# VinAIResearch/Counting-DETR

Measured on AMD Instinct MI355X. Metric: images/sec FSCD-147 2nd-stage train step, higher is better.
Workload: dtype forward bf16x3 (fp32 operands split hi+lo, 3 bf16 MFMAs per product); data / weight gradients bf16 (both operands rounded to bf16, 1 MFMA per product); fp32 accumulate, fp32 storage, fp32 attention softmax / norms / losses / optimizer; 1 GPU; FSCD-147 2nd-stage train step (ResNet-50-DC5 + RCDA enc6/dec6, Q=300 learned, 800x800, T=[37, 120]), fwd+matcher+loss+bwd+clip+AdamW; images_per_gpu=2, global_batch=2, parallelism=dp1, graph=True, precision=bf16x3, precision_backward=bf16, frozen_stage_prefetch=True

## Files before the change

counting_detr_amd/_ffi.py:

```python
import ctypes as C
import os

import torch

_HERE = os.path.dirname(os.path.abspath(__file__))
LIB_PATH = os.environ.get("CDETR_LIB") or os.path.join(_HERE, "lib", "libcdetr_hip.so")

ROWS_DENSE, ROWS_CONV_FWD, ROWS_CONV_DGRAD = 0, 1, 2
_p = C.c_void_p


class ConvGeom(C.Structure):
    _fields_ = [("mode", C.c_int32), ("Ha", C.c_int32), ("Wa", C.c_int32), ("Hc", C.c_int32), ("Wc", C.c_int32),
                ("kh", C.c_int32), ("kw", C.c_int32), ("stride", C.c_int32), ("pad", C.c_int32), ("dil", C.c_int32)]


class GemmDesc(C.Structure):
    _fields_ = [("M", C.c_int32), ("N", C.c_int32), ("K", C.c_int32), ("taps", C.c_int32), ("batch", C.c_int32),
                ("b_layout", C.c_int32), ("relu", C.c_int32), ("precision", C.c_int32), ("out_scale", C.c_float),
                ("A", _p), ("lda", C.c_int64), ("sA", C.c_int64),
                ("B", _p), ("ldb", C.c_int64), ("sB", C.c_int64),
                ("C", _p), ("ldc", C.c_int64), ("sC", C.c_int64),
                ("w_scale", _p), ("bias", _p), ("resid", _p), ("ldr", C.c_int64), ("gate", _p), ("ldg", C.c_int64),
                ("g", ConvGeom), ("B_split", _p), ("batch_inner", C.c_int32), ("flags", C.c_int32),
                ("sA2", C.c_int64), ("sB2", C.c_int64), ("sC2", C.c_int64), ("A16", _p), ("C16", _p),
                ("splitk_ws", _p), ("splitk_ws_bytes", C.c_int64), ("A16lo", _p), ("B16", _p), ("gate16", _p), ("C16lo", _p)]


class WgradDesc(C.Structure):
    _fields_ = [("P", C.c_int32), ("Nout", C.c_int32), ("Cin", C.c_int32), ("taps", C.c_int32), ("batch", C.c_int32), ("precision", C.c_int32),
                ("dY", _p), ("ldy", C.c_int64), ("sY", C.c_int64),
                ("X", _p), ("ldx", C.c_int64), ("sX", C.c_int64),
                ("dW", _p), ("ldw", C.c_int64), ("sW", C.c_int64),
                ("w_scale", _p), ("dbias", _p), ("g", ConvGeom), ("batch_inner", C.c_int32), ("wg_target", C.c_int32),
                ("sY2", C.c_int64), ("sX2", C.c_int64), ("sW2", C.c_int64), ("dY16", _p), ("X16", _p)]


class RcdaFwdDesc(C.Structure):
    _fields_ = [("N", C.c_int32), ("L", C.c_int32), ("H", C.c_int32), ("W", C.c_int32), ("nh", C.c_int32),
                ("precision", C.c_int32), ("scale", C.c_float), ("q_row", _p), ("q_col", _p), ("k_row", _p), ("k_col", _p), ("v", _p),
                ("mask_row", _p), ("mask_col", _p), ("out", _p), ("a_row", _p), ("a_col", _p), ("ws", _p), ("ws_bytes", C.c_int64)]


class RcdaBwdDesc(C.Structure):
    _fields_ = [("N", C.c_int32), ("L", C.c_int32), ("H", C.c_int32), ("W", C.c_int32), ("nh", C.c_int32),
                ("precision", C.c_int32), ("scale", C.c_float), ("d_out", _p), ("a_row", _p), ("a_col", _p), ("v", _p),
                ("ds_row", _p), ("ds_col", _p), ("d_v", _p), ("k_row", _p), ("k_col", _p), ("dq_row", _p), ("dq_col", _p),
                ("q_row", _p), ("q_col", _p), ("dk_row", _p), ("dk_col", _p)]


class AttnDesc(C.Structure):
    _fields_ = [("q", _p), ("k", _p), ("v", _p), ("ldq", C.c_int64), ("ldk", C.c_int64), ("ldv", C.c_int64), ("o", _p), ("lse", _p),
                ("d_o", _p), ("d_q", _p), ("d_k", _p), ("d_v", _p), ("ld_dq", C.c_int64), ("ld_dk", C.c_int64), ("ld_dv", C.c_int64),
                ("work", _p), ("N", C.c_int32), ("Lq", C.c_int32), ("Lk", C.c_int32), ("nh", C.c_int32), ("scale", C.c_float),
                ("precision", C.c_int32)]


class CriterionDesc(C.Structure):
    _fields_ = [("B", C.c_int32), ("Q", C.c_int32), ("C", C.c_int32), ("num_classes", C.c_int32), ("Mmax", C.c_int32), ("alpha", C.c_float),
                ("logits", _p), ("boxes", _p), ("vars", _p), ("tgt_boxes", _p), ("tgt_labels", _p), ("tgt_off", _p), ("idx_i", _p),
                ("idx_j", _p), ("num_boxes", _p), ("losses", _p), ("g_logits", _p), ("g_l1", _p), ("g_giou", _p), ("g_var_box", _p),
                ("g_vars", _p), ("loss_weights", _p)]


class CriterionEvalDesc(C.Structure):
    _fields_ = [("B", C.c_int32), ("Q", C.c_int32), ("C", C.c_int32), ("num_classes", C.c_int32), ("Mmax", C.c_int32), ("alpha", C.c_float),
                ("logits", _p), ("boxes", _p), ("vars", _p), ("tgt_boxes", _p), ("tgt_labels", _p), ("tgt_off", _p), ("idx_i", _p),
                ("idx_j", _p), ("losses", _p), ("loss_weights", _p)]


class MirrorItem(C.Structure):
    _fields_ = [("src", _p), ("dst", _p), ("dst_split", _p), ("scale", _p), ("R", C.c_int32), ("C", C.c_int32), ("taps", C.c_int32),
                ("tile0", C.c_int32), ("transpose", C.c_int32), ("pad_", C.c_int32), ("dst_hi", _p)]


class CocoMatchDesc(C.Structure):
    _fields_ = [("B", C.c_int32), ("A", C.c_int32), ("T", C.c_int32), ("Gtot", C.c_int32), ("Dtot", C.c_int32), ("Gmax", C.c_int32),
                ("gt_boxes", _p), ("gt_area", _p), ("gt_ignore", _p), ("gt_off", _p), ("dt_boxes", _p), ("dt_area", _p), ("dt_off", _p),
                ("iou_thrs", _p), ("area_rng", _p), ("matched", _p), ("det_ignored", _p), ("npig", _p)]


class ImagePrepDesc(C.Structure):
    _fields_ = [("B", C.c_int32), ("Hm", C.c_int32), ("Wm", C.c_int32), ("max_taps", C.c_int32), ("max_rows", C.c_int32), ("pad_", C.c_int32),
                ("pixels", _p), ("pixel_bytes", C.c_int64), ("images", _p), ("tables", _p), ("table_ints", C.c_int64), ("lut", _p),
                ("image", _p), ("mask", _p)]


class EmitDetectionsDesc(C.Structure):
    _fields_ = [("B", C.c_int32), ("Q", C.c_int32), ("N", C.c_int32), ("first", C.c_int32), ("max_det", C.c_int32), ("wire_cap", C.c_int32),
                ("eval_cap", C.c_int32), ("threshold", C.c_float), ("prob", _p), ("boxes", _p), ("points", _p), ("orig_hw", _p), ("counts", _p),
                ("wire_off", _p), ("eval_off", _p), ("wire", _p), ("eval_boxes", _p), ("eval_area", _p), ("eval_score", _p), ("status", _p)]


class EmitPseudoLabelsDesc(C.Structure):
    _fields_ = [("B", C.c_int32), ("R", C.c_int32), ("N", C.c_int32), ("first", C.c_int32), ("max_det", C.c_int32), ("row_cap", C.c_int32),
                ("eval_cap", C.c_int32), ("pad_", C.c_int32), ("points", _p), ("pred_wh", _p), ("counts", _p), ("orig_wh", _p), ("gt_xywh", _p),
                ("img_counts", _p), ("row_off", _p), ("eval_off", _p), ("wire", _p), ("pair_iou", _p), ("eval_boxes", _p), ("eval_area", _p),
                ("eval_score", _p), ("status", _p)]


EXPORTS = ["cdetr_gemm", "cdetr_gemm_dl", "cdetr_gemm_group", "cdetr_wgrad", "cdetr_wgrad_group", "cdetr_colsum", "cdetr_sumsq", "cdetr_adamw_step", "cdetr_adamw_step2", "cdetr_sgd_step", "cdetr_relu_mask", "cdetr_relu_mask2", "cdetr_layernorm_fwd", "cdetr_layernorm_fwd_add", "cdetr_layernorm_bwd", "cdetr_layernorm_bwd_merge", "cdetr_groupnorm_fwd", "cdetr_groupnorm_bwd", "cdetr_groupnorm_fwd_ws", "cdetr_groupnorm_bwd_ws", "cdetr_posadd2",
           "cdetr_hw_reduce", "cdetr_posadd2_hw_reduce", "cdetr_bcast_add2", "cdetr_bcast_add2_sum", "cdetr_add2", "cdetr_grad_merge", "cdetr_sine_embed", "cdetr_sine_embed_bwd", "cdetr_maxpool3x3s2", "cdetr_maxpool3x3s2_split", "cdetr_weight_mirror", "cdetr_weight_images", "cdetr_rcda_fwd", "cdetr_rcda_bwd", "cdetr_mha_fwd", "cdetr_mha_bwd", "cdetr_mha_fwd_lens", "cdetr_mha_bwd_lens", "cdetr_attn_fwd", "cdetr_attn_bwd",
           "cdetr_mask_prep", "cdetr_stem_pack", "cdetr_exemplar_fwd", "cdetr_exemplar_bwd", "cdetr_aggr_weight_fwd", "cdetr_aggr_weight_bwd",
           "cdetr_box_head_fwd", "cdetr_box_head_bwd", "cdetr_match_cost", "cdetr_lsap", "cdetr_criterion_fwd", "cdetr_criterion_bwd", "cdetr_criterion_eval", "cdetr_bbox_criterion_fwd", "cdetr_bbox_criterion_bwd", "cdetr_bbox_criterion_lens_fwd", "cdetr_bbox_criterion_lens_bwd", "cdetr_box_iou_xywh", "cdetr_coco_match", "cdetr_image_prep", "cdetr_emit_detections", "cdetr_emit_pseudo_labels", "cdetr_count_sweep", "cdetr_last_error", "cdetr_abi_version", "cdetr_delay", "cdetr_flag_signal", "cdetr_flag_wait"]

_lib = None


def lib():
    global _lib
    if _lib is None:
        if not os.path.exists(LIB_PATH):
            raise RuntimeError(f"{LIB_PATH} is missing: build it with `python -m counting_detr_amd.build` "
                               "(the Counting-DETR MI355X path has no fallback implementation)")
        L = C.CDLL(LIB_PATH)
        L.cdetr_last_error.restype = C.c_char_p
        L.cdetr_abi_version.restype = C.c_int
        L.cdetr_gemm_dl.restype = C.c_int
        L.cdetr_gemm_dl.argtypes = [_p, C.c_int32, C.c_int32, _p]
        for name in ("cdetr_gemm", "cdetr_wgrad", "cdetr_rcda_fwd", "cdetr_rcda_bwd", "cdetr_attn_fwd", "cdetr_attn_bwd"):
            getattr(L, name).restype = C.c_int
            getattr(L, name).argtypes = [_p, _p]
        L.cdetr_delay.restype = C.c_int
        L.cdetr_delay.argtypes = [C.c_int32, _p]
        L.cdetr_flag_signal.restype = C.c_int
        L.cdetr_flag_signal.argtypes = [_p, _p]
        L.cdetr_flag_wait.restype = C.c_int
        L.cdetr_flag_wait.argtypes = [_p, _p, C.c_int32, C.c_int32, _p]
        L.cdetr_gemm_group.restype = C.c_int
        L.cdetr_gemm_group.argtypes = [_p, C.c_int32, _p]
        L.cdetr_wgrad_group.restype = C.c_int
        L.cdetr_wgrad_group.argtypes = [_p, C.c_int32, _p]
        L.cdetr_colsum.restype = C.c_int
        L.cdetr_colsum.argtypes = [_p, C.c_int64, C.c_int32, C.c_int32, _p, _p]
        L.cdetr_sumsq.restype = C.c_int
        L.cdetr_sumsq.argtypes = [_p, C.c_int64, _p, _p, _p]
        L.cdetr_adamw_step.restype = C.c_int
        L.cdetr_adamw_step.argtypes = [_p, _p, _p, _p, _p, C.c_int64, _p, _p] + [C.c_float] * 6 + [_p]
        L.cdetr_adamw_step2.restype = C.c_int
        L.cdetr_adamw_step2.argtypes = [_p] * 5 + [C.c_float, C.c_float, C.c_int64, C.c_int64, _p, _p] + [C.c_float] * 6 + [_p]
        L.cdetr_sgd_step.restype = C.c_int
        L.cdetr_sgd_step.argtypes = [_p] * 4 + [C.c_float, C.c_float, C.c_int64, C.c_int64, _p, _p] + [C.c_float] * 4 + [_p]
        L.cdetr_relu_mask.restype = C.c_int
        L.cdetr_relu_mask.argtypes = [_p, _p, _p, C.c_int64, C.c_float, _p]
        L.cdetr_relu_mask2.restype = C.c_int
        L.cdetr_relu_mask2.argtypes = [_p, _p, _p, _p, C.c_int64, C.c_float, _p]
        L.cdetr_layernorm_fwd.restype = C.c_int
        L.cdetr_layernorm_fwd.argtypes = [_p] * 6 + [C.c_int32, C.c_int32, C.c_float, _p]
        L.cdetr_layernorm_fwd_add.restype = C.c_int
        L.cdetr_layernorm_fwd_add.argtypes = [_p] * 10 + [C.c_int32, C.c_int32, C.c_float, _p]
        L.cdetr_layernorm_bwd.restype = C.c_int
        L.cdetr_layernorm_bwd.argtypes = [_p] * 9 + [C.c_int32, C.c_int32, _p, _p]
        L.cdetr_layernorm_bwd_merge.restype = C.c_int
        L.cdetr_layernorm_bwd_merge.argtypes = [_p] * 7 + [C.c_float, C.c_float, C.c_int32, C.c_int32] + [_p] * 8 + [C.c_int32, C.c_int32, _p, _p]
        L.cdetr_groupnorm_fwd.restype = C.c_int
        L.cdetr_groupnorm_fwd.argtypes = [_p] * 6 + [C.c_int32] * 4 + [C.c_float, _p]
# ... 108 lines not shown
```

counting_detr_amd/csrc/elementwise.hip:

```cpp
#include "../../include/cdetr_hip.h"
#include "common.h"
#include <stdlib.h>

namespace {

__global__ __launch_bounds__(256) void sumsq_kernel(const float* __restrict__ g, long n, float* __restrict__ ws) {
    float s = 0.f;
    const long n4 = n >> 2;
    const float4* g4 = reinterpret_cast<const float4*>(g);
    for (long i = (long)blockIdx.x * 256 + threadIdx.x; i < n4; i += (long)gridDim.x * 256) {
        const float4 v = g4[i];
        s += v.x * v.x + v.y * v.y + v.z * v.z + v.w * v.w;
    }
    if (blockIdx.x == 0)
        for (long i = (n4 << 2) + threadIdx.x; i < n; i += 256) s += g[i] * g[i];
    s = wave_sum(s);
    __shared__ float part[4];
    if ((threadIdx.x & 63) == 0) part[threadIdx.x >> 6] = s;
    __syncthreads();
    if (threadIdx.x == 0) ws[blockIdx.x] = (part[0] + part[1]) + (part[2] + part[3]);
}

__global__ __launch_bounds__(256) void sumsq_final_kernel(const float* __restrict__ ws, int nblocks, float* __restrict__ out) {
    float t = 0.f;
// ... 72 lines not shown
    if (!clip_coef(sumsq, max_norm, grad_div, coef)) return;
    const long n4 = n >> 2;
    float4* p4 = reinterpret_cast<float4*>(p);
    const float4* g4 = reinterpret_cast<const float4*>(g);
    float4* b4 = reinterpret_cast<float4*>(buf);
    auto upd = [&](float& pp, float gg, float& bb, float l) {
        const float d = gg * coef + wd * pp;
        bb = momentum * bb + d;
        pp -= (l * lr_scale) * bb;
    };
    for (long i = (long)blockIdx.x * 256 + threadIdx.x; i < n4; i += (long)gridDim.x * 256) {
        float4 pp = p4[i], bb = b4[i];
        const float4 gg = g4[i];
        const float4 ll = lr4_at(lr, i, lr0, lr1, lr_split);
        upd(pp.x, gg.x, bb.x, ll.x);
        upd(pp.y, gg.y, bb.y, ll.y);
        upd(pp.z, gg.z, bb.z, ll.z);
        upd(pp.w, gg.w, bb.w, ll.w);
        p4[i] = pp; b4[i] = bb;
    }
    if (blockIdx.x == 0)
        for (long i = (n4 << 2) + threadIdx.x; i < n; i += 256) upd(p[i], g[i], buf[i], lr_at(lr, i, lr0, lr1, lr_split));
}

__global__ void adamw_finish_kernel(const float* __restrict__ sumsq, float* __restrict__ state, float grad_div) {
    const float total_norm = sqrtf(sumsq[0]) * grad_div;
    state[2] = total_norm;
    if (fabsf(total_norm) <= 3.0e38f) state[0] += 1.f;
    else state[3] += 1.f;
}

__global__ __launch_bounds__(256) void relu_mask_kernel(const float* __restrict__ y, const float* __restrict__ dy,
                                                        float* __restrict__ dz, __bf16* __restrict__ dz16, long n, float scale) {
    const long n4 = n >> 2;
    for (long i = (long)blockIdx.x * 256 + threadIdx.x; i < n4; i += (long)gridDim.x * 256) {
        const float4 a = reinterpret_cast<const float4*>(y)[i];
        float4 b = reinterpret_cast<const float4*>(dy)[i];
        b.x = a.x > 0.f ? b.x * scale : 0.f;
        b.y = a.y > 0.f ? b.y * scale : 0.f;
        b.z = a.z > 0.f ? b.z * scale : 0.f;
        b.w = a.w > 0.f ? b.w * scale : 0.f;
        reinterpret_cast<float4*>(dz)[i] = b;
        if (dz16) {
            const f32x2 lo = {b.x, b.y}, hi = {b.z, b.w};
            uint2 t;
            t.x = __builtin_bit_cast(unsigned, __builtin_convertvector(lo, bf16x2));
            t.y = __builtin_bit_cast(unsigned, __builtin_convertvector(hi, bf16x2));
            reinterpret_cast<uint2*>(dz16)[i] = t;
        }
    }
    if (blockIdx.x == 0)
        for (long i = (n4 << 2) + threadIdx.x; i < n; i += 256) {
            const float v = y[i] > 0.f ? dy[i] * scale : 0.f;
            dz[i] = v;
            if (dz16) dz16[i] = (__bf16)v;
        }
}

inline int grid_for(long n4) {
    long b = (n4 + 255) / 256;
    static_assert(CDETR_SUMSQ_MAX_BLOCKS == 2048, "cdetr_sumsq's workspace holds one partial per block of this grid");
    if (b > 2048) b = 2048;
    if (b < 1) b = 1;
    return (int)b;
}


__global__ __launch_bounds__(256) void weight_mirror_kernel(const cdetr_mirror_item* __restrict__ items, const int n_items) {
    __shared__ float tile[32][33];
    const int b = blockIdx.x;
    int lo = 0, hi = n_items - 1;
    while (lo < hi) {
        const int mid = (lo + hi + 1) >> 1;
        if (items[mid].tile0 <= b) lo = mid; else hi = mid - 1;
    }
    const cdetr_mirror_item it = items[lo];
    const int tilesC = (it.C + 31) >> 5, tilesR = (it.R + 31) >> 5;
    int t = b - it.tile0;
    const int tap = t / (tilesR * tilesC);
    t -= tap * tilesR * tilesC;
    const int r0 = (t / tilesC) * 32, c0 = (t % tilesC) * 32;
    const int tx = threadIdx.x & 31, ty = threadIdx.x >> 5;
    __bf16* sp = reinterpret_cast<__bf16*>(it.dst_split);
    float vin[4], sin_[4];
    const int cc = min(c0 + tx, it.C - 1);
#pragma unroll
    for (int p = 0; p < 4; ++p) vin[p] = it.src[((long)min(r0 + ty + 8 * p, it.R - 1) * it.taps + tap) * it.C + cc];
    if (it.scale) {
#pragma unroll
        for (int p = 0; p < 4; ++p) sin_[p] = it.scale[min(r0 + ty + 8 * p, it.R - 1)];
    } else {
#pragma unroll
        for (int p = 0; p < 4; ++p) sin_[p] = 1.f;
    }
#pragma unroll
    for (int p = 0; p < 4; ++p) {
        const int r = r0 + ty + 8 * p, c = c0 + tx;
        const float v = (r < it.R && c < it.C) ? (it.scale ? vin[p] * sin_[p] : vin[p]) : 0.f;
        tile[ty + 8 * p][tx] = v;
        if (!it.transpose && sp && r < it.R && c < it.C) {
            const __bf16 h = (__bf16)v;
            __bf16* g = sp + (long)r * it.taps * it.C * 2 + (long)((tap * it.C + c0) >> 5) * 64;
            g[tx] = h;
            g[32 + tx] = (__bf16)(v - (float)h);
        }
    }
    if (!it.transpose) return;
    __syncthreads();
#pragma unroll
    for (int p = 0; p < 4; ++p) {
        const int c = c0 + ty + 8 * p, r = r0 + tx;
        if (r < it.R && c < it.C) {
            const float v = tile[tx][ty + 8 * p];
            if (it.dst) it.dst[((long)c * it.taps + tap) * it.R + r] = v;
            if (it.dst_hi) reinterpret_cast<__bf16*>(it.dst_hi)[((long)c * it.taps + tap) * it.R + r] = (__bf16)v;
            if (sp) {
                const __bf16 h = (__bf16)v;
                __bf16* g = sp + (long)c * it.taps * it.R * 2 + (long)((tap * it.R + r0) >> 5) * 64;
                g[tx] = h;
                g[32 + tx] = (__bf16)(v - (float)h);
            }
        }
    }
}
constexpr int WIMG_BLOCK = 4096;
__global__ __launch_bounds__(256) void weight_image_kernel(const cdetr_mirror_item* __restrict__ items, const int n_items) {
    const int b = blockIdx.x;
    int lo = 0, hi = n_items - 1;
    while (lo < hi) {
        const int mid = (lo + hi + 1) >> 1;
        if (items[mid].tile0 <= b) lo = mid; else hi = mid - 1;
    }
    const cdetr_mirror_item it = items[lo];
    const long K = (long)it.taps * it.C, total = (long)it.R * K;
    const long e0 = (long)(b - it.tile0) * WIMG_BLOCK + threadIdx.x * 4;
    __bf16* sp = reinterpret_cast<__bf16*>(it.dst_split);
    const bool al = (reinterpret_cast<uintptr_t>(it.src) & 15) == 0;
    float4 v[4];
    float sc[4];
#pragma unroll
    for (int u = 0; u < 4; ++u) {
        const long e = min(e0 + u * 1024, total - 4);
        if (al) v[u] = *reinterpret_cast<const float4*>(it.src + e);
        else v[u] = make_float4(it.src[e], it.src[e + 1], it.src[e + 2], it.src[e + 3]);
        sc[u] = it.scale ? it.scale[e / K] : 1.f;
    }
#pragma unroll
    for (int u = 0; u < 4; ++u) {
        const long e = e0 + u * 1024;
        if (e >= total) continue;
        const float x[4] = {it.scale ? v[u].x * sc[u] : v[u].x, it.scale ? v[u].y * sc[u] : v[u].y, it.scale ? v[u].z * sc[u] : v[u].z,
                            it.scale ? v[u].w * sc[u] : v[u].w};
        __bf16 h[4], l[4];
#pragma unroll
        for (int j = 0; j < 4; ++j) {
            h[j] = (__bf16)x[j];
            l[j] = (__bf16)(x[j] - (float)h[j]);
        }
        __bf16* g = sp + (e >> 5) * 64 + (e & 31);
        *reinterpret_cast<uint2*>(g) = *reinterpret_cast<const uint2*>(h);
        *reinterpret_cast<uint2*>(g + 32) = *reinterpret_cast<const uint2*>(l);
    }
}

template <int NT>
__device__ __forceinline__ float block_sum(float v, float* red) {
    v = wave_sum(v);
    const int lane = threadIdx.x & 63, wid = threadIdx.x >> 6;
    __syncthreads();
    if (lane == 0) red[wid] = v;
    __syncthreads();
    float t = 0.f;
#pragma unroll
    for (int i = 0; i < NT / 64; ++i) t += red[i];
    return t;
}
constexpr int GN_NT = 1024;
constexpr int GN_NT_BWD = 256;

__global__ __launch_bounds__(GN_NT) void gn_fwd_kernel(const float* __restrict__ x, const float* __restrict__ gamma,
                                                     const float* __restrict__ beta, float* __restrict__ y, float* __restrict__ mean,
                                                     float* __restrict__ rstd, int P, int C, int G, float eps) {
    __shared__ float red[GN_NT / 64];
    const int CG = C / G, q4 = CG >> 2;
    const int b = blockIdx.x / G, g = blockIdx.x % G;
    const float* xb = x + (long)b * P * C + g * CG;
    float* yb = y + (long)b * P * C + g * CG;
    const int n4 = P * q4;
    float s1 = 0.f, s2 = 0.f;
    for (int i = threadIdx.x; i < n4; i += GN_NT) {
        const int p = i / q4, c4 = i - p * q4;
        const float4 v = *reinterpret_cast<const float4*>(xb + (long)p * C + c4 * 4);
        s1 += (v.x + v.y) + (v.z + v.w);
    }
    const float inv = 1.f / ((float)P * CG);
    const float mu = block_sum<GN_NT>(s1, red) * inv;
    for (int i = threadIdx.x; i < n4; i += GN_NT) {
        const int p = i / q4, c4 = i - p * q4;
        const float4 v = *reinterpret_cast<const float4*>(xb + (long)p * C + c4 * 4);
        const float a = v.x - mu, b2 = v.y - mu, c2 = v.z - mu, e2 = v.w - mu;
        s2 += (a * a + b2 * b2) + (c2 * c2 + e2 * e2);
// ... 928 lines not shown
```

counting_detr_amd/csrc/igemm.hip:

```cpp
#include "../../include/cdetr_hip.h"
#include "common.h"
#include "rows.h"
#include <stdlib.h>
#include <type_traits>
#include <vector>
#include <algorithm>

namespace {

constexpr int BK = 16;
constexpr int LDS_K = BK + 4;

__device__ __forceinline__ float4 ld4(const float* p) { return *reinterpret_cast<const float4*>(p); }
typedef unsigned u32x4 __attribute__((ext_vector_type(4)));
__device__ __forceinline__ u32x4 ld16(const __bf16* p) { return *reinterpret_cast<const u32x4*>(p); }
__device__ __forceinline__ float4 zero4() { return make_float4(0.f, 0.f, 0.f, 0.f); }

template <int BM, int BN, int BL>
__global__ __launch_bounds__(256) void igemm_kernel(const cdetr_gemm_desc d, const int tilesM, const int vecA,
                                                    const int vecB) {
    constexpr int FM = BM / 64, FN = BN / 64;
    constexpr int A_SLOTS = BM / 64, B_SLOTS = BN / 64;
    constexpr int LDS_N = BN + 4;
    constexpr int B_TILE = (BL == 0) ? BN * LDS_K : BK * LDS_N;
// ... 1518 lines not shown
            const int k = k0 + u * 16 + g4 * 4;
            if constexpr (VA) {
                const float4 t = ld4(arow + (k < kend ? k : 0));
                a[u][0] = t.x; a[u][1] = t.y; a[u][2] = t.z; a[u][3] = t.w;
            } else {
#pragma unroll
                for (int s = 0; s < 4; ++s) a[u][s] = arow[k + s < kend ? k + s : 0];
            }
            if (BL == 0) {
                if constexpr (VB) {
                    const float4 t = ld4(brow + (k < kend ? k : 0));
                    b[u][0] = t.x; b[u][1] = t.y; b[u][2] = t.z; b[u][3] = t.w;
                } else {
#pragma unroll
                    for (int s = 0; s < 4; ++s) b[u][s] = brow[k + s < kend ? k + s : 0];
                }
            } else {
#pragma unroll
                for (int s = 0; s < 4; ++s) {
                    const int kk = k + s < kend ? k + s : 0;
                    b[u][s] = brow[(long)kk * d.ldb];
                    bw[u][s] = wsp[wsc ? kk : 0];
                }
            }
        }
        __builtin_amdgcn_sched_barrier(0);
#pragma unroll
        for (int u = 0; u < UB; ++u) {
            const int k = k0 + u * 16 + g4 * 4;
#pragma unroll
            for (int s = 0; s < 4; ++s) {
                const bool oka = VA ? (k < kend) : (k + s < kend);
                const bool okb = (BL == 0 && VB) ? (k < kend) : (k + s < kend);
                a[u][s] *= oka ? am : 0.f;
                if (BL == 0) b[u][s] *= okb ? bm : 0.f;
                else b[u][s] = (okb && nv) ? (wsc ? b[u][s] * bw[BL == 0 ? 0 : u][s] : b[u][s]) : 0.f;
            }
        }
#pragma unroll
        for (int u = 0; u < UB; ++u)
#pragma unroll
            for (int s = 0; s < 4; ++s) acc = __builtin_amdgcn_mfma_f32_16x16x4f32(a[u][s], b[u][s], acc, 0, 0, 0);
    }
    };
    using T_ = std::true_type;
    using F_ = std::false_type;
    if (vecA) { if (vecB || BL != 0) run(T_{}, T_{}); else run(T_{}, F_{}); }
    else { if (vecB || BL != 0) run(F_{}, T_{}); else run(F_{}, F_{}); }
    mfma_drain(acc);
#pragma unroll
    for (int r = 0; r < 4; ++r) red[wid][r * 64 + lane] = acc[r];
    __syncthreads();
    if (wid != 0) return;
    const int no = tn * 16 + i;
    if (no >= d.N) return;
#pragma unroll
    for (int r = 0; r < 4; ++r) {
        const int mo = tm * 16 + g4 * 4 + r;
        if (mo >= d.M) continue;
        const float sum = (red[0][r * 64 + lane] + red[1][r * 64 + lane]) + (red[2][r * 64 + lane] + red[3][r * 64 + lane]);
        float v = (sum + bias) * d.out_scale + rv[r];
        v = gv[r] > 0.f ? v : 0.f;
        if (d.relu) v = fmaxf(v, 0.f);
        C[(long)mo * d.ldc + no] = v;
        if (C16) C16[(long)mo * d.ldc + no] = (__bf16)v;
    }
}

template <int BL, int UB>
__global__ __launch_bounds__(256) void igemm_direct_kernel(const cdetr_gemm_desc d, const int tilesM, const int tilesN,
                                                           const int vecA, const int vecB) {
    igemm_direct_body<BL, UB>(d, tilesM, tilesN, vecA, vecB, blockIdx.x, blockIdx.z);
}

template <int BL, int UB>
__global__ __launch_bounds__(256) void igemm_direct_group_kernel(const GemmGroupArgs g) {
    int p = 0;
    while (p + 1 < g.n && (int)blockIdx.x >= g.blk0[p + 1]) ++p;
    const GemmGroupItem& it = g.it[p];
    const int lb = blockIdx.x - g.blk0[p];
    igemm_direct_body<BL, UB>(it.d, it.tilesM, it.tilesN, it.vecA, it.vecB, lb % it.nx, lb / it.nx);
}

template <int TERMS>
__global__ __launch_bounds__(512) void igemm_mixed_group_kernel(const GemmGroupArgs g) {
    int p = 0;
    while (p + 1 < g.n && (int)blockIdx.x >= g.blk0[p + 1]) ++p;
    const GemmGroupItem& it = g.it[p];
    const int lb = blockIdx.x - g.blk0[p];
    if (it.pad_ == 0) {
        if (threadIdx.x >= 256) return;
        igemm_direct_body<0, 4>(it.d, it.tilesM, it.tilesN, it.vecA, it.vecB, lb % it.nx, lb / it.nx);
    } else {
        igemm_fast_body<2, 4, 1, 1, 0, 32, 3, TERMS>(it.d, it.tilesM, lb % it.nx, lb / it.nx);
    }
}

__device__ __forceinline__ void wgrad_direct_body(const cdetr_wgrad_desc& d, const int tilesI, const int tilesJ, const int p_per_slice,
                                                  float* __restrict__ dbias, const int bx, const int by, const int bz, const bool single) {
    constexpr int UB = 8;
    const int wid = threadIdx.x >> 6, lane = threadIdx.x & 63;
    const int tile = bx * 4 + wid;
    if (tile >= tilesI * tilesJ) return;
    const int ti = tile % tilesI, tj = tile / tilesI;
    const int i = lane & 15, g4 = lane >> 4;
    const int z = bz;
    const float* __restrict__ dY = d.dY + batch_off(z, d.batch_inner, d.sY, d.sY2);
    const float* __restrict__ X = d.X + batch_off(z, d.batch_inner, d.sX, d.sX2);
    float* __restrict__ dW = d.dW + batch_off(z, d.batch_inner, d.sW, d.sW2);
    const int ci = ti * 16 + i, cc = tj * 16 + i;
    const bool iv = ci < d.Nout, cv = cc < d.Cin;
    const float* ya = dY + (iv ? ci : 0);
    const float* xb = X + (cv ? cc : 0);
    const float fa = iv ? 1.f : 0.f, fb = cv ? 1.f : 0.f;
    const int pbeg = by * p_per_slice, pend = min(d.P, pbeg + p_per_slice);
    float ws[4] = {1.f, 1.f, 1.f, 1.f};
    if (d.w_scale) {
#pragma unroll
        for (int r = 0; r < 4; ++r) ws[r] = d.w_scale[min(ti * 16 + g4 * 4 + r, d.Nout - 1)];
    }
    f32x4 acc = {0.f, 0.f, 0.f, 0.f};
    float bsum = 0.f;
    for (int p0 = pbeg; p0 < pend; p0 += 16 * UB) {
        float a[UB][4], b[UB][4];
#pragma unroll
        for (int u = 0; u < UB; ++u)
#pragma unroll
            for (int s = 0; s < 4; ++s) {
                const int p = p0 + u * 16 + g4 * 4 + s;
                const bool pv = p < pend;
                const long pc = pv ? p : 0;
                a[u][s] = ya[pc * d.ldy] * (pv ? fa : 0.f);
                b[u][s] = xb[pc * d.ldx] * (pv ? fb : 0.f);
            }
#pragma unroll
        for (int u = 0; u < UB; ++u)
#pragma unroll
            for (int s = 0; s < 4; ++s) {
                acc = __builtin_amdgcn_mfma_f32_16x16x4f32(a[u][s], b[u][s], acc, 0, 0, 0);
                bsum += a[u][s];
            }
    }
    mfma_drain(acc);
    const int co = tj * 16 + i;
    if (co < d.Cin) {
#pragma unroll
        for (int r = 0; r < 4; ++r) {
            const int io = ti * 16 + g4 * 4 + r;
            if (io >= d.Nout) continue;
            const float v = acc[r] * ws[r];
            float* dst = dW + (long)io * d.ldw + co;
            if (single) *dst += v;
            else atomicAdd(dst, v);
        }
    }
    if (dbias != nullptr && tj == 0) {
        bsum += __shfl_xor(bsum, 16, 64);
        bsum = xhalf_sum(bsum);
        if (g4 == 0 && iv) atomicAdd(dbias + ci, bsum);
    }
}

__global__ __launch_bounds__(256) void wgrad_direct_kernel(const cdetr_wgrad_desc d, const int tilesI, const int tilesJ,
                                                           const int p_per_slice, float* __restrict__ dbias) {
    wgrad_direct_body(d, tilesI, tilesJ, p_per_slice, dbias, blockIdx.x, blockIdx.y, blockIdx.z, gridDim.y == 1);
}
// ... 284 lines not shown
        const int tilesM = (d.M + 15) / 16, tilesN = (d.N + 15) / 16;
        dim3 grid(tilesM * tilesN, 1, d.batch);
        const int cpw = (((d.K + 15) >> 4) + 3) >> 2;
        auto go = [&](auto k0, auto k1) {
            if (d.b_layout == 0) hipLaunchKernelGGL(k0, grid, dim3(256), 0, st, d, tilesM, tilesN, vecA, vecB);
            else hipLaunchKernelGGL(k1, grid, dim3(256), 0, st, d, tilesM, tilesN, vecA, vecB);
        };
        if (cpw <= 4) go(igemm_direct_kernel<0, 4>, igemm_direct_kernel<1, 4>);
        else if (cpw <= 8) go(igemm_direct_kernel<0, 8>, igemm_direct_kernel<1, 8>);
        else go(igemm_direct_kernel<0, 16>, igemm_direct_kernel<1, 16>);
        return cdetr_launch_status("cdetr_gemm");
    }
    if (vecA && vecB && (d.K % 32) == 0) {
        if (gemm_is_f44(d)) {
            if (d.splitk_ws && d.batch == 1 && blocks(128, 128) < 224 && (long)d.K * d.taps >= 4096) return launch_gemm_fast<2, 4, 2, 1, 32>(d, st);
            if (blocks(128, 128) < 224 && blocks(96, 128) <= 256) return launch_gemm_fast<3, 4, 1, 1, 32>(d, st);
            return launch_gemm_fast<4, 4, 1, 1, 32>(d, st);
        }
        if (gemm_is_f24(d)) return launch_gemm_fast<2, 4, 1, 1, 32>(d, st);
        if ((d.K % 64) == 0 && blocks(64, 64) < 512) return launch_gemm_fast<2, 2, 1, 1, 64>(d, st);
        return launch_gemm_fast<2, 2, 1, 1, 32>(d, st);
    }
    if (d.N > 64 && d.M > 64 && blocks(128, 128) >= 384) return launch_gemm<128, 128>(d, st, vecA, vecB);
    if (d.M > 64 && blocks(128, 64) >= 384) return launch_gemm<128, 64>(d, st, vecA, vecB);
    return launch_gemm<64, 64>(d, st, vecA, vecB);
}

extern "C" int cdetr_gemm_group(const cdetr_gemm_desc* descs, int32_t n, void* stream) {
    CDETR_CHECK_ARG(n >= 0 && (descs != nullptr || n == 0), "cdetr_gemm_group: bad arguments");
    hipStream_t st = reinterpret_cast<hipStream_t>(stream);
    const char* force_s = cdetr_tune_env("CDETR_GEMM_VARIANT");
    const bool grouping = !(force_s && atoi(force_s) != 0);
    std::vector<int> cls[5];
    for (int i = 0; i < n; ++i) {
        const cdetr_gemm_desc& d = descs[i];
        if (int rcv = check_gemm_desc(d)) return rcv;
        if (d.M == 0) continue;
        const int vecA = gemm_vec_a(d), vecB = gemm_vec_b(d);
        int c = -1;
        if (grouping && gemm_is_direct(d, vecA, vecB)) {
            if (d.b_layout == 0) {
                const int cpw = (((d.K + 15) >> 4) + 3) >> 2;
                c = cpw <= 4 ? 0 : (cpw <= 8 ? 1 : 2);
            }
        } else if (grouping && vecA && vecB && (d.K % 32) == 0 && !gemm_is_f44(d) && gemm_is_f24(d) && d.B_split && d.batch == 1) {
            c = d.precision == 3 ? 4 : 3;
        }
        if (c >= 0) cls[c].push_back(i);
        else if (int rc1 = cdetr_gemm(&d, stream)) return rc1;
    }
    const int tc = !cls[3].empty() ? 3 : 4;
    if (!cls[0].empty() && (cls[3].empty() != cls[4].empty()) && cls[0].size() + cls[tc].size() <= (size_t)GG_MAX) {
        GemmGroupArgs g;
        int m = 0;
        g.blk0[0] = 0;
        for (int pass = 0; pass < 2; ++pass) {
            for (int idx : (pass == 0 ? cls[tc] : cls[0])) {
                GemmGroupItem& it = g.it[m];
                it.d = descs[idx];
                it.vecA = gemm_vec_a(it.d); it.vecB = gemm_vec_b(it.d); it.pad_ = pass == 0 ? 1 : 0;
                if (pass == 1) {
                    it.tilesM = (it.d.M + 15) / 16; it.tilesN = (it.d.N + 15) / 16;
                    it.nx = it.tilesM * it.tilesN;
                } else {
                    it.tilesM = (it.d.M + 63) / 64; it.tilesN = (it.d.N + 127) / 128;
                    it.nx = 8 * ((it.tilesM + 7) / 8) * it.tilesN;
                }
                g.blk0[m + 1] = g.blk0[m] + it.nx * it.d.batch;
                ++m;
            }
        }
        g.n = m;
        const int bytes = (2 * 64 * 36 + 2 * 128 * 36) * 4;
        if (tc == 3) {
            if (int rcl = raise_lds(igemm_mixed_group_kernel<3>, bytes, "cdetr_gemm_group")) return rcl;
            hipLaunchKernelGGL(igemm_mixed_group_kernel<3>, dim3(g.blk0[m]), dim3(512), bytes, st, g);
        } else {
            if (int rcl = raise_lds(igemm_mixed_group_kernel<1>, bytes, "cdetr_gemm_group")) return rcl;
            hipLaunchKernelGGL(igemm_mixed_group_kernel<1>, dim3(g.blk0[m]), dim3(512), bytes, st, g);
        }
        if (int rcl = cdetr_launch_status("cdetr_gemm_group")) return rcl;
        cls[0].clear();
        cls[tc].clear();
    }
    for (int c = 0; c < 5; ++c) {
        for (size_t c0 = 0; c0 < cls[c].size(); c0 += GG_MAX) {
            const int m = (int)std::min<size_t>(GG_MAX, cls[c].size() - c0);
            if (m == 1) { if (int rc1 = cdetr_gemm(&descs[cls[c][c0]], stream)) return rc1; continue; }
            GemmGroupArgs g;
            g.n = m; g.blk0[0] = 0;
            for (int k = 0; k < m; ++k) {
                GemmGroupItem& it = g.it[k];
                it.d = descs[cls[c][c0 + k]];
                it.vecA = gemm_vec_a(it.d); it.vecB = gemm_vec_b(it.d); it.pad_ = 0;
                if (c < 3) {
                    it.tilesM = (it.d.M + 15) / 16; it.tilesN = (it.d.N + 15) / 16;
                    it.nx = it.tilesM * it.tilesN;
                } else {
                    it.tilesM = (it.d.M + 63) / 64; it.tilesN = (it.d.N + 127) / 128;
                    it.nx = 8 * ((it.tilesM + 7) / 8) * it.tilesN;
                }
                g.blk0[k + 1] = g.blk0[k] + it.nx * it.d.batch;
            }
            if (c == 0) hipLaunchKernelGGL((igemm_direct_group_kernel<0, 4>), dim3(g.blk0[m]), dim3(256), 0, st, g);
            else if (c == 1) hipLaunchKernelGGL((igemm_direct_group_kernel<0, 8>), dim3(g.blk0[m]), dim3(256), 0, st, g);
            else if (c == 2) hipLaunchKernelGGL((igemm_direct_group_kernel<0, 16>), dim3(g.blk0[m]), dim3(256), 0, st, g);
            else if (c == 3) {
                const int bytes = (2 * 64 * 36 + 2 * 128 * 36) * 4;
                if (int rcl = raise_lds(igemm_fast_group_kernel<2, 4, 1, 1, 0, 32, 3>, bytes, "cdetr_gemm_group")) return rcl;
                hipLaunchKernelGGL((igemm_fast_group_kernel<2, 4, 1, 1, 0, 32, 3>), dim3(g.blk0[m]), dim3(512), bytes, st, g);
            } else {
                const int bytes = (2 * 64 * 36 + 2 * 128 * 36) * 4;
                if (int rcl = raise_lds(igemm_fast_group_kernel<2, 4, 1, 1, 0, 32, 3, 1>, bytes, "cdetr_gemm_group")) return rcl;
                hipLaunchKernelGGL((igemm_fast_group_kernel<2, 4, 1, 1, 0, 32, 3, 1>), dim3(g.blk0[m]), dim3(512), bytes, st, g);
            }
            if (int rcl = cdetr_launch_status("cdetr_gemm_group")) return rcl;
        }
    }
    return CDETR_OK;
}

namespace {
bool wgrad_has_twins(const cdetr_wgrad_desc& d);
bool wgrad_is_direct(const cdetr_wgrad_desc& d);
bool wgrad_is_fast(const cdetr_wgrad_desc& d);
int check_wgrad_desc(const cdetr_wgrad_desc& d) {
    CDETR_CHECK_ARG(d.P >= 0 && d.Nout > 0 && d.Cin > 0 && d.taps > 0 && d.batch > 0, "cdetr_wgrad: bad sizes");
    CDETR_CHECK_ARG((d.dY || d.dY16) && (d.X || d.X16) && d.dW, "cdetr_wgrad: null pointer");
    CDETR_CHECK_ARG((d.dY && d.X) || (wgrad_has_twins(d) && wgrad_is_fast(d) && !wgrad_is_direct(d)),
                    "cdetr_wgrad: dY == NULL / X == NULL need dY16 + X16, plain-bf16 products and a problem of the tile-kernel class");
    CDETR_CHECK_ARG(aligned16(d.dY) && aligned16(d.X) && (d.sY & 3) == 0 && (d.sX & 3) == 0 && (d.sY2 & 3) == 0 && (d.sX2 & 3) == 0, "cdetr_wgrad: dY/X must be 16-byte aligned");
    if (d.g.mode == CDETR_ROWS_DENSE) {
        CDETR_CHECK_ARG(d.taps == 1, "cdetr_wgrad: dense rows need taps == 1");
    } else {
        CDETR_CHECK_ARG(d.g.mode == CDETR_ROWS_CONV_FWD && d.taps == d.g.kh * d.g.kw, "cdetr_wgrad: geometry");
        CDETR_CHECK_ARG(d.P % (d.g.Hc * d.g.Wc) == 0, "cdetr_wgrad: P is not images*Hc*Wc");
    }
    return CDETR_OK;
}
void direct_wgrad_plan(const cdetr_wgrad_desc& d, int& tilesI, int& tilesJ, int& per, int& slices) {
    tilesI = (d.Nout + 15) / 16; tilesJ = (d.Cin + 15) / 16;
    slices = (d.P + 127) / 128;
    if (slices > 8) slices = 8;
    per = (d.P + slices - 1) / slices;
    per = ((per + 15) / 16) * 16;
    slices = (d.P + per - 1) / per;
}
bool wgrad_is_direct(const cdetr_wgrad_desc& d) {
    return d.g.mode == CDETR_ROWS_DENSE && (d.P <= 256 || !((d.ldy & 3) == 0 && (d.ldx & 3) == 0 && (d.Nout & 3) == 0 && (d.Cin & 3) == 0)) && d.P <= 1024;
}
bool wgrad_has_twins(const cdetr_wgrad_desc& d) {
    return d.precision == 3 && d.dY16 && d.X16 && !d.dbias && (d.Nout & 7) == 0 && (d.Cin & 7) == 0 && (d.ldy & 7) == 0 && (d.ldx & 7) == 0 &&
           (d.sY & 7) == 0 && (d.sX & 7) == 0 && (d.sY2 & 7) == 0 && (d.sX2 & 7) == 0 && aligned16(d.dY16) && aligned16(d.X16) && d.Nout >= 8 && d.Cin >= 8;
}
int wgrad_kp() {
    const char* e = cdetr_tune_env("CDETR_WGRAD_KP");
    const int kp = e ? atoi(e) : 1;
    return kp >= 4 ? 4 : kp >= 2 ? 2 : 1;
}
bool wgrad_is_fast(const cdetr_wgrad_desc& d) { return (d.ldy & 3) == 0 && (d.ldx & 3) == 0 && (d.Nout & 3) == 0 && (d.Cin & 3) == 0; }
}

extern "C" int cdetr_wgrad(const cdetr_wgrad_desc* dp, void* stream) {
    CDETR_CHECK_ARG(dp != nullptr, "cdetr_wgrad: null descriptor");
    cdetr_wgrad_desc d = *dp;
    if (int rcv = check_wgrad_desc(d)) return rcv;
// ... 224 lines not shown
```

counting_detr_amd/csrc/rcda.hip:

```cpp
#include "../../include/cdetr_hip.h"
#include "common.h"
#include <algorithm>
#include <type_traits>
#include <stdlib.h>

namespace {

__device__ __forceinline__ void xcd_slab(int& bx, int& by) {
    const int gx = gridDim.x, total = gx * gridDim.y;
    if (total & 7) return;
    const int lin = by * gx + bx;
    const int l2 = (lin & 7) * (total >> 3) + (lin >> 3);
    by = l2 / gx;
    bx = l2 - by * gx;
}


constexpr int D = 32;
constexpr int QW = 32;

__device__ __forceinline__ float4 ld4(const float* p) { return *reinterpret_cast<const float4*>(p); }

struct FwdSmem {
    int sw, sh;
// ... 879 lines not shown
        if (!PROBE && nq > 0 && d.ds_col) save_rows(Acol, sm.sh, d.ds_col + (((long)n * d.nh + head) * L + qbase) * Hp, nq, Hp, lane);
    }
    stamp(3);
    float qv[2][2][8];
    if (PREC == 1 && d.dq_row && d.dk_row) {
#pragma unroll
        for (int side = 0; side < 2; ++side)
#pragma unroll
            for (int st = 0; st < 2; ++st)
#pragma unroll
                for (int j = 0; j < 8; ++j) {
                    const int qq = qbase + 16 * st + 8 * g + j;
                    qv[side][st][j] = (side == 0 ? d.q_row : d.q_col)[((long)n * L + min(max(qq, 0), L - 1)) * E + head * D + i32];
                }
    }
    if (d.dq_row) {
        float* Kk = smem + sm.off_kk;
        if (kpre_ok) {
#pragma unroll
            for (int u = 0; u < KP; ++u) {
                const int idx = tid + NT * u;
                if (idx < nk8) *reinterpret_cast<float4*>(Kk + (idx >> 3) * D + (idx & 7) * 4) = kpre[u];
            }
        } else
        for (int base = 0; base < nk8; base += 4 * NT) {
            float4 t[4];
#pragma unroll
            for (int u = 0; u < 4; ++u) {
                const int idx = min(base + tid + NT * u, nk8 - 1);
                const int key = idx >> 3, c4 = idx & 7;
                const float* src = (key < W) ? d.k_row + ((long)n * W + key) * E + head * D + c4 * 4
                                             : d.k_col + ((long)n * H + (key - W)) * E + head * D + c4 * 4;
                t[u] = ld4(src);
            }
#pragma unroll
            for (int u = 0; u < 4; ++u) {
                const int idx = base + tid + NT * u;
                if (idx < nk8) *reinterpret_cast<float4*>(Kk + (idx >> 3) * D + (idx & 7) * 4) = t[u];
            }
        }
        __syncthreads();
        stamp(4);
        if constexpr (PREC == 1) {
#pragma unroll
            for (int side = 0; side < 2; ++side) {
                const int nkeys = side == 0 ? W : H;
                const float* S = side == 0 ? dArow + i32 * sm.sw : Acol + i32 * sm.sh;
                const float* Ks = Kk + (side == 0 ? 0 : W * D) + i32;
                f32x16 acc = {0.f, 0.f, 0.f, 0.f, 0.f, 0.f, 0.f, 0.f, 0.f, 0.f, 0.f, 0.f, 0.f, 0.f, 0.f, 0.f};
                const int nks = (nkeys + 15) >> 4;
                for (int st = 0; st < nks; ++st) {
                    float a[8], b[8];
#pragma unroll
                    for (int j = 0; j < 8; ++j) {
                        const int w = 16 * st + 8 * g + j;
                        const int wc = min(w, nkeys - 1);
                        const float av = Ks[wc * D], bv = S[wc];
                        a[j] = (w < nkeys) ? av : 0.f;
                        b[j] = (w < nkeys) ? bv : 0.f;
                    }
                    bf16x8 ah, al, bh, bl;
                    split_bf16x8(a, ah, al);
                    split_bf16x8(b, bh, bl);
                    acc = mfma_bf16_terms<TERMS>(ah, al, bh, bl, acc);
                }
                mfma_drain(acc);
                if (qvalid) {
                    float* dst = (side == 0 ? d.dq_row : d.dq_col) + ((long)n * L + q) * E + head * D + 4 * g;
#pragma unroll
                    for (int j = 0; j < 4; ++j)
                        *reinterpret_cast<float4*>(dst + 8 * j) = make_float4(acc[4 * j], acc[4 * j + 1], acc[4 * j + 2], acc[4 * j + 3]);
                }
            }
            stamp(5);
            if (d.dk_row) {
                const bool wg_reduce = W <= 128 && H <= 128;
                constexpr int NTL = 4;
#pragma unroll
                for (int side = 0; side < 2; ++side) {
                    const int nkeys = side == 0 ? W : H;
                    const float* S = side == 0 ? dArow : Acol;
                    float* Sw = side == 0 ? dArow : Acol;
                    const int sstr = side == 0 ? sm.sw : sm.sh;
                    float* acc_g = (side == 0 ? d.dk_row + (long)n * W * E : d.dk_col + (long)n * H * E) + head * D + i32;
                    bf16x8 bh[2], bl[2];
#pragma unroll
                    for (int st = 0; st < 2; ++st) {
                        float b[8];
#pragma unroll
                        for (int j = 0; j < 8; ++j) b[j] = (qbase + 16 * st + 8 * g + j < L) ? qv[side][st][j] : 0.f;
                        split_bf16x8(b, bh[st], bl[st]);
                    }
                    const int ntile = (nkeys + 31) >> 5;
                    auto tile = [&](int tl) __attribute__((always_inline)) -> f32x16 {
                        const int wkey = 32 * tl + i32, wc = min(wkey, nkeys - 1);
                        f32x16 acc = {0.f, 0.f, 0.f, 0.f, 0.f, 0.f, 0.f, 0.f, 0.f, 0.f, 0.f, 0.f, 0.f, 0.f, 0.f, 0.f};
#pragma unroll
                        for (int st = 0; st < 2; ++st) {
                            float a[8];
#pragma unroll
                            for (int j = 0; j < 8; ++j) {
                                const float av = S[(16 * st + 8 * g + j) * sstr + wc];
                                a[j] = (wkey < nkeys) ? av : 0.f;
                            }
                            bf16x8 ah, al;
                            split_bf16x8(a, ah, al);
                            acc = mfma_bf16_terms<TERMS>(ah, al, bh[st], bl[st], acc);
                        }
                        mfma_drain(acc);
                        return acc;
                    };
                    if (wg_reduce) {
                        f32x16 accs[NTL];
#pragma unroll
                        for (int tl = 0; tl < NTL; ++tl)
                            if (tl < ntile) accs[tl] = tile(tl);
                        wave_sync();
#pragma unroll
                        for (int tl = 0; tl < NTL; ++tl)
                            if (tl < ntile) {
#pragma unroll
                                for (int r = 0; r < 16; ++r) {
                                    const int wk = 32 * tl + (r & 3) + 8 * (r >> 2) + 4 * g;
                                    Sw[min(wk, nkeys) * D + i32] = accs[tl][r];
                                }
                            }
                    } else {
                        for (int tl = 0; tl < ntile; ++tl) {
                            const f32x16 acc = tile(tl);
#pragma unroll
                            for (int r = 0; r < 16; ++r) {
                                const int wk = 32 * tl + (r & 3) + 8 * (r >> 2) + 4 * g;
                                if (wk < nkeys) atomicAdd(acc_g + (long)wk * E, acc[r]);
                            }
                        }
                    }
                }
                if (wg_reduce) {
                    __syncthreads();
                    const int nrow = W * D, ntot = (W + H) * D;
                    for (int e = tid; e < ntot; e += NT) {
                        const bool rowside = e < nrow;
                        const int idx = rowside ? e : e - nrow;
                        const float* base = rowside ? smem + sm.off_r + idx : smem + sm.off_u + idx;
                        const int wstr = rowside ? QW * sm.sw : QW * sm.su;
                        float sum = 0.f;
#pragma unroll
                        for (int wv = 0; wv < NW; ++wv) sum += base[wv * wstr];
                        const int key = idx >> 5, ch = idx & 31;
                        float* dst = rowside ? d.dk_row + ((long)n * W + key) * E + head * D + ch : d.dk_col + ((long)n * H + key) * E + head * D + ch;
                        atomicAdd(dst, sum);
                    }
                }
            }
            stamp(6);
            flush_probe();
            return;
        }
#pragma unroll
        for (int side = 0; side < 2; ++side) {
            const int nkeys = side == 0 ? W : H;
            const float* S = side == 0 ? dArow + i32 * sm.sw : Acol + i32 * sm.sh;
            const float* Ks = Kk + (side == 0 ? 0 : W * D) + 16 * g;
            float acc[16];
#pragma unroll
            for (int j = 0; j < 16; ++j) acc[j] = 0.f;
#pragma unroll 2
            for (int k = 0; k < nkeys; ++k) {
                const float a = S[k];
#pragma unroll
                for (int c4 = 0; c4 < 4; ++c4) {
                    const float4 kv = *reinterpret_cast<const float4*>(Ks + k * D + c4 * 4);
                    acc[c4 * 4 + 0] = fmaf(a, kv.x, acc[c4 * 4 + 0]);
                    acc[c4 * 4 + 1] = fmaf(a, kv.y, acc[c4 * 4 + 1]);
                    acc[c4 * 4 + 2] = fmaf(a, kv.z, acc[c4 * 4 + 2]);
                    acc[c4 * 4 + 3] = fmaf(a, kv.w, acc[c4 * 4 + 3]);
                }
            }
            if (qvalid) {
                float* dst = (side == 0 ? d.dq_row : d.dq_col) + ((long)n * L + q) * E + head * D + 16 * g;
#pragma unroll
                for (int c4 = 0; c4 < 4; ++c4)
                    *reinterpret_cast<float4*>(dst + c4 * 4) = make_float4(acc[c4 * 4], acc[c4 * 4 + 1], acc[c4 * 4 + 2], acc[c4 * 4 + 3]);
            }
        }
    }
}

template <int NF, int NW, int PREC, int TERMS = 3, bool PROBE = false>
__global__ __launch_bounds__(64 * NW) void rcda_bwd_kernel(const cdetr_rcda_bwd_desc d) {
    int bx_ = blockIdx.x, by_ = blockIdx.y;
    xcd_slab(bx_, by_);
    rcda_bwd_body<NF, NW, PREC, TERMS, PROBE>(d, bx_, by_);
}

template <int NF, int PREC>
__global__ __launch_bounds__(256) void rcda_dv_kernel(const cdetr_rcda_bwd_desc d, const int q_per_slice) {
    constexpr int QT = 64;
    constexpr int HR = 32 * NF;
    extern __shared__ __attribute__((aligned(16))) float smem[];
    const int H = d.H, W = d.W, L = d.L, E = d.nh * D;
    const int Wp = (W + 3) & ~3, Hp = (H + 7) & ~7;
    float* Ac = smem;
    float* Ar = Ac + QT * HR;
    float* Do = Ar + QT * Wp;
    const int tid = threadIdx.x, lane = tid & 63, wid = tid >> 6;
    const int i32 = lane & 31, g = lane >> 5;
    const int n = blockIdx.y / d.nh, head = blockIdx.y % d.nh;
    const int w = blockIdx.x * 4 + wid;
    const bool wvalid = w < W;
    const int qs = blockIdx.z * q_per_slice;
    const int qe = min(L, qs + q_per_slice);
    const float* gac = d.a_col + ((long)n * d.nh + head) * L * Hp;
    const float* gar = d.a_row + ((long)n * d.nh + head) * L * Wp;
    const float* gdo = d.d_out + (long)n * L * E + head * D;

    f32x16 acc[NF];
#pragma unroll
    for (int f = 0; f < NF; ++f)
#pragma unroll
        for (int r = 0; r < 16; ++r) acc[f][r] = 0.f;

    for (int q0 = qs; q0 < qe; q0 += QT) {
        const int nq = min(QT, qe - q0);
        __syncthreads();
        for (int idx = tid; idx < QT * HR; idx += 256) {
            const int r = idx / HR, c = idx - r * HR;
            Ac[idx] = (r < nq && c < Hp) ? gac[(long)(q0 + r) * Hp + c] : 0.f;
        }
        for (int idx = tid; idx < QT * Wp; idx += 256) {
            const int r = idx / Wp;
            Ar[idx] = (r < nq) ? gar[(long)q0 * Wp + idx] : 0.f;
        }
        for (int idx = tid; idx < QT * 8; idx += 256) {
            const int r = idx >> 3, c4 = idx & 7;
            *reinterpret_cast<float4*>(Do + r * D + c4 * 4) =
                (r < nq) ? ld4(gdo + (long)(q0 + r) * E + c4 * 4) : make_float4(0.f, 0.f, 0.f, 0.f);
        }
        __syncthreads();
        if (wvalid && PREC == 0) {
#pragma unroll 2
            for (int kk = 0; kk < QT / 8; ++kk) {
#pragma unroll
                for (int s = 0; s < 4; ++s) {
                    const int qq = kk * 8 + g * 4 + s;
                    const float ar = Ar[qq * Wp + w];
                    const float b = Do[qq * D + i32];
#pragma unroll
                    for (int f = 0; f < NF; ++f) {
                        const float a = Ac[qq * HR + 32 * f + i32] * ar;
                        acc[f] = __builtin_amdgcn_mfma_f32_32x32x2f32(a, b, acc[f], 0, 0, 0);
                    }
                }
            }
        }
        if (wvalid && PREC == 1) {
#pragma unroll 2
            for (int kp = 0; kp < QT / 16; ++kp) {
                float arv[8], bv[8];
                int qs[8];
#pragma unroll
                for (int t = 0; t < 4; ++t) {
                    qs[t] = (2 * kp) * 8 + g * 4 + t;
                    qs[4 + t] = (2 * kp + 1) * 8 + g * 4 + t;
                }
#pragma unroll
                for (int t = 0; t < 8; ++t) {
                    arv[t] = Ar[qs[t] * Wp + w];
                    bv[t] = Do[qs[t] * D + i32];
                }
                bf16x8 bh, bl;
                split_bf16x8(bv, bh, bl);
#pragma unroll
                for (int f = 0; f < NF; ++f) {
                    float av[8];
#pragma unroll
                    for (int t = 0; t < 8; ++t) av[t] = Ac[qs[t] * HR + 32 * f + i32] * arv[t];
                    bf16x8 ah, al;
                    split_bf16x8(av, ah, al);
                    acc[f] = mfma_bf16x3(ah, al, bh, bl, acc[f]);
                }
            }
        }
    }
    mfma_drain(acc);
    if (!wvalid) return;
#pragma unroll
    for (int f = 0; f < NF; ++f)
#pragma unroll
        for (int r = 0; r < 16; ++r) {
            const int h = 32 * f + (r & 3) + 8 * (r >> 2) + 4 * g;
            if (h < H) atomicAdd(d.d_v + (((long)n * H + h) * W + w) * E + head * D + i32, acc[f][r]);
        }
}

struct Dv2Smem { int art, dot, act, tile, total; };
__host__ __device__ inline Dv2Smem dv2_smem() {
    Dv2Smem s;
    s.art = 0;
    s.dot = 64 * 68;
    s.act = s.dot + 32 * 68;
    s.tile = s.act + 8 * 68;
    s.total = 2 * s.tile;
    return s;
}

template <int TERMS = 3>
__device__ __forceinline__ void rcda_dv2_body(const cdetr_rcda_bwd_desc& d, const int q_per_slice, const int bx, const int by, const int bz) {
    constexpr int QT = 64, ARS = 136;
    extern __shared__ __attribute__((aligned(16))) float smem[];
    const Dv2Smem sm = dv2_smem();
    const int H = d.H, W = d.W, L = d.L, E = d.nh * D;
    const int Wp = (W + 3) & ~3, Hp = (H + 7) & ~7;
    const int tid = threadIdx.x, lane = tid & 63, wid = tid >> 6;
    const int i32 = lane & 31, g = lane >> 5;
    const int n = by / d.nh, head = by % d.nh;
    const int nhg = (H + 7) >> 3;
    const int wchunk = bx / nhg;
    const int nwc = (Wp + 63) >> 6;
    const int wper = (((Wp + nwc - 1) / nwc) + 3) & ~3;
    const int wbase = wchunk * wper;
    const int Wc = min(wper, Wp - wbase);
    const int h0 = (bx - wchunk * nhg) * 8, h = h0 + wid;
    const int qs = bz * q_per_slice;
    const int qe = min(L, qs + q_per_slice);
    const int ntile = (qe - qs + QT - 1) / QT;
    if (ntile <= 0) return;

    const int nrb = 16 * (Wc >> 2);
    int role, q4, x4;
    if (tid < nrb) { role = 0; q4 = tid & 15; x4 = tid >> 4; }
    else if (tid >= 256 && tid < 384) { role = 1; q4 = (tid - 256) & 15; x4 = (tid - 256) >> 4; }
    else if (tid >= 384 && tid < 416) { role = 2; q4 = (tid - 384) & 15; x4 = (tid - 384) >> 4; }
    else { role = 3; q4 = 0; x4 = 0; }
    const float* src;
    long rstride;
    if (role == 0) { src = d.a_row + (((long)n * d.nh + head) * L) * Wp + wbase + x4 * 4; rstride = Wp; }
    else if (role == 1) { src = d.d_out + (long)n * L * E + head * D + x4 * 4; rstride = E; }
    else { src = d.a_col + (((long)n * d.nh + head) * L) * Hp + min(h0 + x4 * 4, Hp - 4); rstride = Hp; }
    float4 rs[2][4];
    unsigned rmask[2] = {0, 0};
    int tf = 0;
    auto fetch = [&](float4 (&r)[4], unsigned& m) __attribute__((always_inline)) {
        const int qb = qs + min(tf, ntile - 1) * QT + q4 * 4;
        m = 0;
#pragma unroll
        for (int kk = 0; kk < 4; ++kk) {
            const int q = qb + kk;
            r[kk] = ld4(src + (long)min(q, L - 1) * rstride);
            m |= (q < qe ? 1u : 0u) << kk;
        }
        ++tf;
    };
    auto stash = [&](const float4 (&r0)[4], unsigned m, int buf) __attribute__((always_inline)) {
        float4 r[4];
#pragma unroll
        for (int kk = 0; kk < 4; ++kk) r[kk] = ((m >> kk) & 1u) ? r0[kk] : make_float4(0.f, 0.f, 0.f, 0.f);
        float* base = smem + buf * sm.tile;
        if (role == 0) {
            __bf16* dst = reinterpret_cast<__bf16*>(base + sm.art) + (x4 * 4) * ARS + q4 * 4;
            stash_split4(dst, 64, r[0].x, r[1].x, r[2].x, r[3].x);
            stash_split4(dst + ARS, 64, r[0].y, r[1].y, r[2].y, r[3].y);
            stash_split4(dst + 2 * ARS, 64, r[0].z, r[1].z, r[2].z, r[3].z);
            stash_split4(dst + 3 * ARS, 64, r[0].w, r[1].w, r[2].w, r[3].w);
        } else if (role == 1 || role == 2) {
            float* dst = base + (role == 1 ? sm.dot : sm.act) + (x4 * 4) * 68 + q4 * 4;
            *reinterpret_cast<float4*>(dst) = make_float4(r[0].x, r[1].x, r[2].x, r[3].x);
            *reinterpret_cast<float4*>(dst + 68) = make_float4(r[0].y, r[1].y, r[2].y, r[3].y);
            *reinterpret_cast<float4*>(dst + 2 * 68) = make_float4(r[0].z, r[1].z, r[2].z, r[3].z);
            *reinterpret_cast<float4*>(dst + 3 * 68) = make_float4(r[0].w, r[1].w, r[2].w, r[3].w);
        }
    };
    for (int idx = tid; idx < 2 * (64 - Wc) * (ARS / 2); idx += 512) {
        const int b = idx / ((64 - Wc) * (ARS / 2)), r = idx - b * (64 - Wc) * (ARS / 2);
        smem[b * sm.tile + sm.art + Wc * (ARS / 2) + r] = 0.f;
    }

    f32x16 acc[2];
#pragma unroll
    for (int f = 0; f < 2; ++f)
#pragma unroll
        for (int r = 0; r < 16; ++r) acc[f][r] = 0.f;

    auto compute = [&](int buf) __attribute__((always_inline)) {
        const float* base = smem + buf * sm.tile;
        const __bf16* art = reinterpret_cast<const __bf16*>(base + sm.art) + i32 * ARS + 8 * g;
        const float* dot = base + sm.dot + i32 * 68 + 8 * g;
        const float* act = base + sm.act + wid * 68 + 8 * g;
#pragma unroll
        for (int ks = 0; ks < 4; ++ks) {
            const float4 d0 = *reinterpret_cast<const float4*>(dot + 16 * ks), d1 = *reinterpret_cast<const float4*>(dot + 16 * ks + 4);
            const float4 a0 = *reinterpret_cast<const float4*>(act + 16 * ks), a1 = *reinterpret_cast<const float4*>(act + 16 * ks + 4);
            const float x[8] = {d0.x * a0.x, d0.y * a0.y, d0.z * a0.z, d0.w * a0.w, d1.x * a1.x, d1.y * a1.y, d1.z * a1.z, d1.w * a1.w};
            bf16x8 bh, bl;
            split_bf16x8(x, bh, bl);
#pragma unroll
            for (int f = 0; f < 2; ++f) {
                const bf16x8 ah = *reinterpret_cast<const bf16x8*>(art + 32 * f * ARS + 16 * ks);
                const bf16x8 al = *reinterpret_cast<const bf16x8*>(art + 32 * f * ARS + 64 + 16 * ks);
                acc[f] = mfma_bf16_terms<TERMS>(ah, al, bh, bl, acc[f]);
            }
        }
    };

    fetch(rs[0], rmask[0]);
    fetch(rs[1], rmask[1]);
    __syncthreads();
    stash(rs[0], rmask[0], 0);
    __syncthreads();
    int t = 0;
    for (; t + 1 < ntile; t += 2) {
        fetch(rs[0], rmask[0]);
        compute(0);
        stash(rs[1], rmask[1], 1);
        __syncthreads();
        fetch(rs[1], rmask[1]);
        compute(1);
        stash(rs[0], rmask[0], 0);
        __syncthreads();
    }
    if (t < ntile) compute(0);
    mfma_drain(acc);
    if (h >= H) return;
#pragma unroll
    for (int f = 0; f < 2; ++f)
#pragma unroll
        for (int r = 0; r < 16; ++r) {
            const int wl = 32 * f + (r & 3) + 8 * (r >> 2) + 4 * g, w = wbase + wl;
            if (wl < Wc && w < W) atomicAdd(d.d_v + (((long)n * H + h) * W + w) * E + head * D + i32, acc[f][r]);
        }
}

template <int TERMS = 3>
__global__ __launch_bounds__(512) void rcda_dv2_kernel(const cdetr_rcda_bwd_desc d, const int q_per_slice) {
    int bx_ = blockIdx.x, by_ = blockIdx.y;
    xcd_slab(bx_, by_);
    rcda_dv2_body<TERMS>(d, q_per_slice, bx_, by_, blockIdx.z);
}

template <int NF, int NW, int TERMS>
__global__ __launch_bounds__(512) void rcda_bwd_all_kernel(const cdetr_rcda_bwd_desc d, const int nqb, const int hgroups, const int q_per_slice) {
    int bx_ = blockIdx.x, by_ = blockIdx.y;
    xcd_slab(bx_, by_);
    if (bx_ < nqb) {
        if ((int)threadIdx.x >= 64 * NW) return;
        rcda_bwd_body<NF, NW, 1, TERMS>(d, bx_, by_);
    } else {
        const int t = bx_ - nqb;
        rcda_dv2_body<TERMS>(d, q_per_slice, t % hgroups, by_, t / hgroups);
    }
}

template <typename F>
int set_smem(F func, int bytes, const char* what) {
    if (bytes > 160 * 1024) {
        cdetr_set_error("%s: needs %d bytes of LDS (> 160 KiB): feature map too large for this tiling", what, bytes);
        return CDETR_ERR_UNSUPPORTED;
    }
    if (bytes > 64 * 1024) {
        hipError_t e = hipFuncSetAttribute(reinterpret_cast<const void*>(func), hipFuncAttributeMaxDynamicSharedMemorySize, bytes);
        if (e != hipSuccess) {
            cdetr_set_error("%s: hipFuncSetAttribute(%d): %s", what, bytes, hipGetErrorString(e));
            return CDETR_ERR_LAUNCH;
        }
    }
    return CDETR_OK;
}

template <int NF>
int launch_rcda_fwd(const cdetr_rcda_fwd_desc& d, hipStream_t st) {
    constexpr int NW = 4;
    const FwdSmem sm = fwd_smem(d.H, d.W, NW);
    const int bytes = sm.total * 4;
    int rc;
    dim3 grid((d.L + QW * NW - 1) / (QW * NW), d.N * d.nh), block(64 * NW);
    if (d.precision == 1) {
        if ((rc = set_smem(rcda_fwd_kernel<NF, NW, 1>, bytes, "cdetr_rcda_fwd"))) return rc;
        hipLaunchKernelGGL((rcda_fwd_kernel<NF, NW, 1>), grid, block, bytes, st, d);
    } else {
        if ((rc = set_smem(rcda_fwd_kernel<NF, NW, 0>, bytes, "cdetr_rcda_fwd"))) return rc;
        hipLaunchKernelGGL((rcda_fwd_kernel<NF, NW, 0>), grid, block, bytes, st, d);
    }
    return cdetr_launch_status("cdetr_rcda_fwd");
}
template <int NF, int NW>
int launch_rcda_bwd_all(const cdetr_rcda_bwd_desc& d, hipStream_t st, int hgroups, int slices, int per) {
    const int bytes = std::max(bwd_smem(d.H, d.W, NF, NW, d.dq_row != nullptr).total * 4, dv2_smem().total * 4);
    int rc;
    const int nqb = (d.L + QW * NW - 1) / (QW * NW);
    dim3 grid(nqb + hgroups * slices, d.N * d.nh);
    if (d.precision == 3) {
        if ((rc = set_smem(rcda_bwd_all_kernel<NF, NW, 1>, bytes, "cdetr_rcda_bwd"))) return rc;
        hipLaunchKernelGGL((rcda_bwd_all_kernel<NF, NW, 1>), grid, dim3(512), bytes, st, d, nqb, hgroups, per);
    } else {
        if ((rc = set_smem(rcda_bwd_all_kernel<NF, NW, 3>, bytes, "cdetr_rcda_bwd"))) return rc;
        hipLaunchKernelGGL((rcda_bwd_all_kernel<NF, NW, 3>), grid, dim3(512), bytes, st, d, nqb, hgroups, per);
    }
    return cdetr_launch_status("cdetr_rcda_bwd(dS+dV)");
}
template <int NF, int NW>
int launch_rcda_bwd(const cdetr_rcda_bwd_desc& d, hipStream_t st) {
    const BwdSmem sm = bwd_smem(d.H, d.W, NF, NW, d.dq_row != nullptr);
    const int bytes = sm.total * 4;
    int rc;
    dim3 grid((d.L + QW * NW - 1) / (QW * NW), d.N * d.nh), block(64 * NW);
    if constexpr (NF == 4) {
        if (d.precision == 3) {
            if ((rc = set_smem(rcda_bwd_kernel<NF, NW, 1, 1>, bytes, "cdetr_rcda_bwd"))) return rc;
            hipLaunchKernelGGL((rcda_bwd_kernel<NF, NW, 1, 1>), grid, block, bytes, st, d);
            return cdetr_launch_status("cdetr_rcda_bwd(dS)");
        }
        if (d.precision >= 1) {
            if ((rc = set_smem(rcda_bwd_kernel<NF, NW, 1>, bytes, "cdetr_rcda_bwd"))) return rc;
            hipLaunchKernelGGL((rcda_bwd_kernel<NF, NW, 1>), grid, block, bytes, st, d);
            return cdetr_launch_status("cdetr_rcda_bwd(dS)");
        }
    }
    if ((rc = set_smem(rcda_bwd_kernel<NF, NW, 0>, bytes, "cdetr_rcda_bwd"))) return rc;
    hipLaunchKernelGGL((rcda_bwd_kernel<NF, NW, 0>), grid, block, bytes, st, d);
    return cdetr_launch_status("cdetr_rcda_bwd(dS)");
}
inline bool rcda_wg5(int L, int NH) {
    const long wg4 = (long)((L + QW * 4 - 1) / (QW * 4)) * NH, wg5 = (long)((L + QW * 5 - 1) / (QW * 5)) * NH;
    return wg4 > 256 && wg4 <= 512 && wg5 <= 256;
}
inline int fwd2_slices(const cdetr_rcda_fwd_desc& d, int base, int nt, int lds_bytes) {
    if (!d.ws || base > RCDA_WS_COUNTERS) return 1;
    int hs;
    const char* f = cdetr_tune_env("CDETR_RCDA_HS");
    if (f) hs = atoi(f);
    else {
        const int per_cu = lds_bytes > 0 ? std::max(1, std::min(4, (160 * 1024) / lds_bytes)) : 1;
        (void)per_cu;
        hs = 256 / base;
    }
    hs = std::min(std::min(hs, 8), d.H / 8);
    const long avail = (long)d.ws_bytes - (long)RCDA_WS_COUNTERS * 4;
    while (hs > 1 && (long)base * hs * 16 * nt * 4 > avail) --hs;
    return hs < 1 ? 1 : hs;
}
inline int rcda_probe() {
    const char* p = cdetr_tune_env("CDETR_RCDA_PROBE");
    return p ? atoi(p) : 0;
}

}

extern "C" int cdetr_rcda_fwd(const cdetr_rcda_fwd_desc* dp, void* stream) {
    CDETR_CHECK_ARG(dp != nullptr, "cdetr_rcda_fwd: null descriptor");
    const cdetr_rcda_fwd_desc d = *dp;
    CDETR_CHECK_ARG(d.N > 0 && d.L > 0 && d.H > 0 && d.W > 0 && d.nh > 0, "cdetr_rcda_fwd: bad sizes");
    CDETR_CHECK_ARG(d.H <= 128 && d.W <= 1024, "cdetr_rcda_fwd: H must be <= 128 (got %d)", d.H);
    CDETR_CHECK_ARG(d.q_row && d.q_col && d.k_row && d.k_col && d.v && d.out, "cdetr_rcda_fwd: null pointer");
    CDETR_CHECK_ARG((d.a_row != nullptr) == (d.a_col != nullptr), "cdetr_rcda_fwd: a_row and a_col are saved together or not at all (both NULL: inference)");
    hipStream_t st = reinterpret_cast<hipStream_t>(stream);
    if (d.precision == 1 && d.W <= 96) {
        const int ks = (d.W + 15) / 16;
        auto go = [&](auto kern, int NWv, int KSv = 0, bool sliced = true) -> int {
            const FwdSmem sm = fwd_smem(d.H, d.W, NWv);
            const int bytes = fwd2_smem(sm, d.H, d.W, KSv ? KSv : ks).total * 4;
            int rc;
            if ((rc = set_smem(kern, bytes, "cdetr_rcda_fwd"))) return rc;
            dim3 grid((d.L + QW * NWv - 1) / (QW * NWv), d.N * d.nh), block(64 * NWv);
            if (sliced) grid.z = fwd2_slices(d, (int)(grid.x * grid.y), 64 * NWv, bytes);
            hipLaunchKernelGGL(kern, grid, block, bytes, st, d);
            return cdetr_launch_status("cdetr_rcda_fwd");
        };
        if (const int probe = rcda_probe(); probe && d.ws && ks == 4 && d.H <= 64)
            return probe == 5 ? go(rcda_fwd2_kernel<5, 4, 2, true>, 5, 0, false) : go(rcda_fwd2_kernel<4, 4, 2, true>, 4, 0, false);
        if (ks == 4 && rcda_wg5(d.L, d.N * d.nh)) return go(rcda_fwd2_kernel<5, 4>, 5);
        if (ks > 4 || d.H > 64) {
            if (d.H > 64 && d.H <= 96) return ks <= 4 ? go(rcda_fwd2_kernel<4, 4, 3>, 4, 4) : go(rcda_fwd2_kernel<4, 6, 3>, 4, 6);
            if (ks <= 4) return go(rcda_fwd2_kernel<4, 4>, 4, 4);
            return ks == 5 ? go(rcda_fwd2_kernel<4, 5>, 4) : go(rcda_fwd2_kernel<4, 6>, 4);
        }
        if (ks == 1) return go(rcda_fwd2_kernel<4, 1>, 4);
        if (ks == 2) return go(rcda_fwd2_kernel<4, 2>, 4);
        if (ks == 3) return go(rcda_fwd2_kernel<4, 3>, 4);
        return go(rcda_fwd2_kernel<4, 4>, 4);
    }
    if (d.H <= 32) return launch_rcda_fwd<1>(d, st);
    if (d.H <= 64) return launch_rcda_fwd<2>(d, st);
    return launch_rcda_fwd<4>(d, st);
}

extern "C" int cdetr_rcda_bwd(const cdetr_rcda_bwd_desc* dp, void* stream) {
    CDETR_CHECK_ARG(dp != nullptr, "cdetr_rcda_bwd: null descriptor");
    const cdetr_rcda_bwd_desc d = *dp;
    CDETR_CHECK_ARG(d.N > 0 && d.L > 0 && d.H > 0 && d.W > 0 && d.nh > 0, "cdetr_rcda_bwd: bad sizes");
    CDETR_CHECK_ARG(d.H <= 128 && d.W <= 1024, "cdetr_rcda_bwd: H must be <= 128 (got %d)", d.H);
    CDETR_CHECK_ARG(d.d_out && d.a_row && d.a_col && d.v && d.d_v, "cdetr_rcda_bwd: null pointer");
    CDETR_CHECK_ARG((d.ds_row && d.ds_col) || (!d.ds_row && !d.ds_col && d.dk_row),
                    "cdetr_rcda_bwd: ds_row / ds_col may only be omitted (both) when the fused q / k gradients are requested");
    CDETR_CHECK_ARG(!d.dq_row || (d.dq_col && d.k_row && d.k_col), "cdetr_rcda_bwd: dq_row needs dq_col, k_row and k_col");
    CDETR_CHECK_ARG(!d.dk_row || (d.dq_row && d.dk_col && d.q_row && d.q_col && d.precision >= 1),
                    "cdetr_rcda_bwd: dk_row needs dk_col, q_row, q_col, the dq_* outputs and a split-bf16 precision (1 or 3)");
    hipStream_t st = reinterpret_cast<hipStream_t>(stream);
    const int NF = d.H <= 32 ? 1 : (d.H <= 64 ? 2 : 4);
    const int Wp = (d.W + 3) & ~3;
    int rc;
    if (const int probe = rcda_probe(); probe && NF == 2 && d.precision == 3 && d.ds_row && d.dk_row) {
        const int NWp = probe == 5 ? 5 : 4;
        const BwdSmem sm = bwd_smem(d.H, d.W, 2, NWp, true);
        dim3 grid((d.L + QW * NWp - 1) / (QW * NWp), d.N * d.nh), block(64 * NWp);
        if (NWp == 5) {
            if ((rc = set_smem(rcda_bwd_kernel<2, 5, 1, 1, true>, sm.total * 4, "cdetr_rcda_bwd"))) return rc;
            hipLaunchKernelGGL((rcda_bwd_kernel<2, 5, 1, 1, true>), grid, block, sm.total * 4, st, d);
        } else {
            if ((rc = set_smem(rcda_bwd_kernel<2, 4, 1, 1, true>, sm.total * 4, "cdetr_rcda_bwd"))) return rc;
            hipLaunchKernelGGL((rcda_bwd_kernel<2, 4, 1, 1, true>), grid, block, sm.total * 4, st, d);
        }
        return cdetr_launch_status("cdetr_rcda_bwd(probe)");
    }
    const bool wg5 = NF == 2 && rcda_wg5(d.L, d.N * d.nh);
    const bool dv2 = d.precision >= 1;
    if (dv2) {
        const int hgroups = ((d.H + 7) / 8) * ((Wp + 63) / 64);
        const long base = (long)hgroups * d.N * d.nh;
        const long ds_wgs = (long)((d.L + QW * 4 - 1) / (QW * 4)) * d.N * d.nh;
        const int dv2_target = ds_wgs <= 128 ? 112 : 224;
        int slices = (int)((dv2_target + base - 1) / base);
        const int max_slices = (d.L + 255) / 256;
        if (slices > max_slices) slices = max_slices;
        if (slices < 1) slices = 1;
        int per = (d.L + slices - 1) / slices;
        per = ((per + 63) / 64) * 64;
        slices = (d.L + per - 1) / per;
        if (NF == 1) return launch_rcda_bwd_all<1, 4>(d, st, hgroups, slices, per);
        if (NF == 2) return wg5 ? launch_rcda_bwd_all<2, 5>(d, st, hgroups, slices, per) : launch_rcda_bwd_all<2, 4>(d, st, hgroups, slices, per);
        if ((rc = launch_rcda_bwd<4, 4>(d, st))) return rc;
        const int bytes = dv2_smem().total * 4;
        if (d.precision == 3) {
            if ((rc = set_smem(rcda_dv2_kernel<1>, bytes, "cdetr_rcda_bwd(dV)"))) return rc;
            hipLaunchKernelGGL(rcda_dv2_kernel<1>, dim3(hgroups, d.N * d.nh, slices), dim3(512), bytes, st, d, per);
        } else {
            if ((rc = set_smem(rcda_dv2_kernel<3>, bytes, "cdetr_rcda_bwd(dV)"))) return rc;
            hipLaunchKernelGGL(rcda_dv2_kernel<3>, dim3(hgroups, d.N * d.nh, slices), dim3(512), bytes, st, d, per);
        }
        return cdetr_launch_status("cdetr_rcda_bwd(dV)");
    }
    if (NF == 1) rc = launch_rcda_bwd<1, 4>(d, st);
    else if (NF == 2) rc = wg5 ? launch_rcda_bwd<2, 5>(d, st) : launch_rcda_bwd<2, 4>(d, st);
    else rc = launch_rcda_bwd<4, 4>(d, st);
    if (rc) return rc;
    const int bytes = (64 * 32 * NF + 64 * Wp + 64 * 32) * 4;
    const int wgroups = (d.W + 3) / 4;
    const long base = (long)wgroups * d.N * d.nh;
    int slices = (int)((1024 + base - 1) / base);
    const int max_slices = (d.L + 127) / 128;
    if (slices > max_slices) slices = max_slices;
    if (slices < 1) slices = 1;
    int per = (d.L + slices - 1) / slices;
    per = ((per + 63) / 64) * 64;
    slices = (d.L + per - 1) / per;
    dim3 grid(wgroups, d.N * d.nh, slices), block(256);
    auto dv = [&](auto kern) -> int {
        if ((rc = set_smem(kern, bytes, "cdetr_rcda_bwd(dV)"))) return rc;
        hipLaunchKernelGGL(kern, grid, block, bytes, st, d, per);
        return cdetr_launch_status("cdetr_rcda_bwd(dV)");
    };
    if (NF == 1) return dv(rcda_dv_kernel<1, 0>);
    if (NF == 2) return dv(rcda_dv_kernel<2, 0>);
    return dv(rcda_dv_kernel<4, 0>);
}
```

counting_detr_amd/engine.py:

```python
import math
import os
import sys

import torch
import torch.distributed as dist

from . import backbone as _bb
from .misc import NestedTensor, get_world_size, is_dist_avail_and_initialized, nested_tensor_from_tensor_list, reduce_dict

UNUSED_PREFIXES = ("input_proj.",)


def _segment_of(name):
    if "backbone" in name:
        for li in (4, 3, 2):
            if f"layer{li}." in name:
                return {4: 1, 3: 2, 2: 3}[li]
        return 3
    return 0


class FlatGradExchange:

    def __init__(self, flat_g, seg_bounds):
# ... 77 lines not shown
                if g is not None:
                    g.replay()
                else:
                    self.works.append(dist.all_reduce(buf, async_op=True))
        elif self.stream is not None:
            ev = torch.cuda.Event()
            ev.record(torch.cuda.current_stream())
            self.stream.wait_event(ev)
            if also is not None:
                self.stream.wait_stream(also)
            with torch.cuda.stream(self.stream):
                b0 = mark(self.stream)
                if g is not None:
                    g.replay()
                else:
                    dist.all_reduce(buf)
                b1 = mark(self.stream)
            if self.trace is not None:
                self.trace["buckets"].append((seg, b0, b1))
        else:
            dist.all_reduce(buf)

    def finish(self):
        nseg = len(self.seg_bounds) - 1
        for seg in range(nseg):
            if seg not in self.launched:
                self.segment_done(seg)
        self.launched = []
        if self.stream is not None:
            cur = torch.cuda.current_stream()
            if self.on_side:
                ea = eb = None
                if self.probe is not None:
                    ea, eb = torch.cuda.Event(enable_timing=True), torch.cuda.Event(enable_timing=True)
                    ea.record(cur)
                for w in self.works:
                    w.wait()
                self.works = []
                if self._pg_stream is not None:
                    cur.wait_stream(self._pg_stream)
                cur.wait_stream(self.stream)
                if ea is not None:
                    eb.record(cur)
                    self.probe.append((ea, eb))
                return
            if self.probe is not None:
                ea, eb = torch.cuda.Event(enable_timing=True), torch.cuda.Event(enable_timing=True)
                ea.record(cur)
                eb.record(self.stream)
                self.probe.append((ea, eb))
            cur.wait_stream(self.stream)

    def exposed_ms(self):
        if not self.probe:
            return None
        return [max(0.0, ea.elapsed_time(eb)) for ea, eb in self.probe]


def build_weight_mirror(model, named, dgrad=True):
    from . import ops
    entries, fwd, seen = [], [], set()
    for m in model.modules():
        if isinstance(m, _bb.Bottleneck):
            pairs = [(m.conv1, m.bn1), (m.conv2, m.bn2), (m.conv3, m.bn3)]
            if m.downsample is not None:
                pairs.append((m.downsample[0], m.downsample[1]))
            for conv, bn in pairs:
                w = conv.weight.data
                seen.add(w.data_ptr())
                if not w.is_cuda:
                    continue
                if conv.weight.requires_grad and dgrad:
                    entries.append((w, bn.affine()[0]))
                if w.shape[1] % 32 == 0:
                    fwd.append((w, bn.affine()[0]))
    for _, p in named:
        if p.data_ptr() in seen or not p.is_cuda or min(p.shape[:2] if p.dim() >= 2 else (0,)) < 32:
            continue
        if p.dim() == 2 or (p.dim() == 4 and p.shape[2] == 1 and p.shape[3] == 1):
            if dgrad:
                entries.append((p.data, None))
            if p.shape[1] % 32 == 0:
                fwd.append((p.data, None))
    return ops.WeightMirror(entries, fwd) if (entries or fwd) else None


class _DeviceEvents:
    DISABLE_TIMING, RELEASE_TO_DEVICE = 0x2, 0x40000000

    def __init__(self, n=64):
        import ctypes
        self._c = ctypes
        self._hip = ctypes.CDLL("libamdhip64.so")
        self._hip.hipEventCreateWithFlags.argtypes = [ctypes.POINTER(ctypes.c_void_p), ctypes.c_uint]
        self._hip.hipEventRecord.argtypes = [ctypes.c_void_p, ctypes.c_void_p]
        self._hip.hipStreamWaitEvent.argtypes = [ctypes.c_void_p, ctypes.c_void_p, ctypes.c_uint]
        self._hip.hipEventDestroy.argtypes = [ctypes.c_void_p]
        self._ring = []
        for _ in range(n):
            h = ctypes.c_void_p()
            rc = self._hip.hipEventCreateWithFlags(ctypes.byref(h), self.DISABLE_TIMING | self.RELEASE_TO_DEVICE)
            if rc != 0:
                raise RuntimeError(f"hipEventCreateWithFlags failed ({rc})")
            self._ring.append(h)
        self._i = 0

    def record(self, stream):
        h = self._ring[self._i]
        self._i = (self._i + 1) % len(self._ring)
        rc = self._hip.hipEventRecord(h, self._c.c_void_p(stream.cuda_stream))
        if rc != 0:
            raise RuntimeError(f"hipEventRecord failed ({rc})")
        return h

    def wait(self, stream, h):
        rc = self._hip.hipStreamWaitEvent(self._c.c_void_p(stream.cuda_stream), h, 0)
        if rc != 0:
            raise RuntimeError(f"hipStreamWaitEvent failed ({rc})")

    def order(self, later, earlier):
        self.wait(later, self.record(earlier))

    def __del__(self):
        try:
            for h in self._ring:
                self._hip.hipEventDestroy(h)
        except Exception:
            pass


class _TorchEvents:

    def record(self, stream):
        ev = torch.cuda.Event()
        ev.record(stream)
        return ev

    def wait(self, stream, ev):
        stream.wait_event(ev)

    def order(self, later, earlier):
        later.wait_stream(earlier)


def _scoped(fn):
    import functools

    @functools.wraps(fn)
    def wrapper(self, *a, **k):
        from . import ops
        with ops.arithmetic(*self.arith):
            return fn(self, *a, **k)
    return wrapper


def model_unused_prefixes(model):
    return tuple(f"{n}.{p}" for n, m in model.named_modules() if n for p in getattr(m, "unused_prefixes", ()))


class Trainer:
    unused_prefixes = UNUSED_PREFIXES

    def __init__(self, model, criterion, args, device=None, precision=None, precision_bwd=None):
        from . import ops as _ops
        self.arith = (int(_ops.PRECISION if precision is None else precision), int(_ops.PRECISION_BWD if precision_bwd is None else precision_bwd))
        self.model, self.criterion, self.args = model, criterion, args
        self.device = torch.device(device or args.device)
# ... 1443 lines not shown
```

counting_detr_amd/ops.py:

```python
import os

import torch

from . import _ffi
from ._ffi import CriterionDesc, MirrorItem, ConvGeom, GemmDesc, RcdaBwdDesc, RcdaFwdDesc, WgradDesc, check, lib, ptr, stream_ptr

import ctypes as C


PROFILE = None

import os as _os
PRECISION = int(_os.environ.get("CDETR_PRECISION", "1"))
PRECISION_BWD = int(_os.environ.get("CDETR_PRECISION_BWD", "3"))
MHA_BWD_BF16 = _os.environ.get("CDETR_MHA_BWD_BF16", "0") == "1"


def bwd_precision():
    return PRECISION_BWD if PRECISION == 1 else PRECISION


class arithmetic:

    def __init__(self, precision, precision_bwd=None):
# ... 288 lines not shown
        self.event = self.side.record_event()
        return self.ctx.__exit__(*exc)

    def join(self):
        torch.cuda.current_stream().wait_event(self.event)


def colsum_(X2d, out):
    M, N = X2d.shape
    check(lib().cdetr_colsum(ptr(X2d), X2d.stride(0), M, N, ptr(out), stream_ptr()), "cdetr_colsum")


def relu_mask(y, dy, scale=1.0, twin=False):
    dy = dy.contiguous()
    dz = torch.empty_like(dy)
    if twin:
        dz16 = torch.empty(dy.shape, device=dy.device, dtype=torch.bfloat16)
        check(lib().cdetr_relu_mask2(ptr(y), ptr(dy), ptr(dz), ptr(dz16), dy.numel(), scale, stream_ptr()), "cdetr_relu_mask2")
        return dz, dz16
    check(lib().cdetr_relu_mask(ptr(y), ptr(dy), ptr(dz), dy.numel(), scale, stream_ptr()), "cdetr_relu_mask")
    return dz


def split_groups(x):
    hi = x.bfloat16()
    lo = (x - hi.float()).bfloat16()
    sh = x.shape[:-1] + (x.shape[-1] // 32, 32)
    return torch.cat([hi.view(sh), lo.view(sh)], dim=-1).contiguous()


class Groups:
    __slots__ = ("t", "shape")

    def __init__(self, t, shape):
        self.t, self.shape = t, tuple(shape)

    @classmethod
    def empty(cls, shape, device):
        assert shape[-1] % 32 == 0
        return cls(torch.empty(tuple(shape[:-1]) + (shape[-1] // 32, 64), device=device, dtype=torch.bfloat16), shape)

    @classmethod
    def of(cls, x):
        return cls(split_groups(x), x.shape)

    @property
    def device(self):
        return self.t.device

    @property
    def is_cuda(self):
        return self.t.is_cuda

    def float(self):
        g = self.t.float()
        return (g[..., :32] + g[..., 32:]).reshape(self.shape)


GROUPS = os.environ.get("CDETR_GROUPS", "0") != "0"
GROUPS_MIN_ROWS = 4096


def use_groups(rows, channels):
    return GROUPS and PRECISION == 1 and MIRROR is not None and rows >= GROUPS_MIN_ROWS and channels % 64 == 0


def split_planes(x):
    hi = x.to(torch.bfloat16)
    return hi, (x - hi.float()).to(torch.bfloat16)


def bf16_twins():
    return TWINS and bwd_precision() == 3


def grad_buffer(p):
    if p.grad is None:
        p.grad = torch.zeros_like(p)
    return p.grad


class WeightMirror:

    def __init__(self, entries, fwd_entries=()):
        import bisect
        import numpy as np
        self._bisect = bisect
        dev = (entries or fwd_entries)[0][0].device
        tot_t = sum(w.numel() for w, _ in entries)
        tot_f = sum(w.numel() for w, _ in fwd_entries)
        self.flat = torch.zeros(max(tot_t, 1), device=dev, dtype=torch.float32)
        self.flat_ts = torch.zeros(max(tot_t, 1), device=dev, dtype=torch.float32)
        self.flat_t16 = torch.zeros(max(tot_t, 1), device=dev, dtype=torch.bfloat16)
        self.flat_fs = torch.zeros(max(tot_f, 1), device=dev, dtype=torch.float32)
        self._keep = []
        items = (MirrorItem * (len(entries) + len(fwd_entries)))()
        self.t_entries, self.f_entries = [], []
        tile0 = 0
        self.nT = len(entries)

        def geom(w):
            R, Cc = w.shape[0], w.shape[1]
            taps = w.shape[2] * w.shape[3] if w.dim() == 4 else 1
            if w.dim() == 4:
                assert taps == 1 or w.is_contiguous(memory_format=torch.channels_last)
            else:
                assert w.is_contiguous()
            return R, Cc, taps

        off = 0
        for i, (w, sc) in enumerate(entries):
            R, Cc, taps = geom(w)
            it = items[i]
            it.src, it.dst = w.data_ptr(), self.flat.data_ptr() + 4 * off
            has_split = R % 32 == 0
            it.dst_split = (self.flat_ts.data_ptr() + 4 * off) if has_split else None
            it.dst_hi = self.flat_t16.data_ptr() + 2 * off
            it.scale = sc.data_ptr() if sc is not None else None
            it.R, it.C, it.taps, it.tile0, it.transpose = R, Cc, taps, tile0, 1
            self.t_entries.append((w.data_ptr(), w.numel() * 4, off, R, Cc, taps, sc.data_ptr() if sc is not None else 0, has_split))
            self._keep.append((w, sc))
            tile0 += ((R + 31) // 32) * ((Cc + 31) // 32) * taps
            off += w.numel()
        self.tilesT = tile0
        tile0 = 0
        off = 0
        for j, (w, sc) in enumerate(fwd_entries):
            R, Cc, taps = geom(w)
            assert Cc % 32 == 0
            it = items[len(entries) + j]
            it.src, it.dst, it.dst_split = w.data_ptr(), None, self.flat_fs.data_ptr() + 4 * off
            it.scale = sc.data_ptr() if sc is not None else None
            it.R, it.C, it.taps, it.tile0, it.transpose = R, Cc, taps, tile0, 0
            self.f_entries.append((w.data_ptr(), w.numel() * 4, off, R, Cc, taps, sc.data_ptr() if sc is not None else 0, True))
            self._keep.append((w, sc))
            tile0 += (w.numel() + 4095) // 4096
            off += w.numel()
        self.tilesF, self.nF = tile0, len(fwd_entries)
        raw = np.frombuffer(bytes(items), dtype=np.uint8).copy()
        self.items_dev = torch.from_numpy(raw).to(dev)
        self.item_bytes = C.sizeof(MirrorItem)
        self.t_entries.sort()
        self.f_entries.sort()
        self._tb = [e[0] for e in self.t_entries]
        self._fb = [e[0] for e in self.f_entries]
        self._memo_t, self._memo_f = {}, {}

    def refresh(self, part="all"):
        if part in ("all", "fwd") and self.nF:
            check(lib().cdetr_weight_images(self.items_dev.data_ptr() + self.nT * self.item_bytes, self.nF, self.tilesF, stream_ptr()),
                  "cdetr_weight_images")
        if part in ("all", "bwd") and self.nT:
            check(lib().cdetr_weight_mirror(self.items_dev.data_ptr(), self.nT, self.tilesT, stream_ptr()), "cdetr_weight_mirror")

    def _find(self, table, bases, w, scale):
        p = w.data_ptr()
        i = self._bisect.bisect_right(bases, p) - 1
        if i < 0:
            return None
        e = table[i]
        if p >= e[0] + e[1] or e[6] != (scale.data_ptr() if scale is not None else 0):
            return None
        row0 = (p - e[0]) // (4 * e[4] * e[5])
        if (p - e[0]) != row0 * 4 * e[4] * e[5] or (row0 and e[5] != 1):
            return None
        return e, row0

    def lookup(self, w, scale=None):
        key = (w.data_ptr(), scale.data_ptr() if scale is not None else 0)
        hit = self._memo_t.get(key, False)
        if hit is not False:
            return hit
        r = self._find(self.t_entries, self._tb, w, scale)
        if r is None:
            out = None
        else:
            (base, nbytes, off, R, Cc, taps, sptr, has_split), row0 = r
            sp = self.flat_ts[off + row0:] if (has_split and row0 % 32 == 0) else None
            out = (self.flat[off + row0:], taps * R, sp, self.flat_t16[off + row0:] if row0 % 8 == 0 else None)
        self._memo_t[key] = out
        return out

    def lookup_fwd(self, w, scale=None):
        key = (w.data_ptr(), scale.data_ptr() if scale is not None else 0)
        hit = self._memo_f.get(key, False)
        if hit is not False:
            return hit
        r = self._find(self.f_entries, self._fb, w, scale)
        if r is None:
            out = None
        else:
            (base, nbytes, off, R, Cc, taps, sptr, _), row0 = r
            out = self.flat_fs[off + row0 * Cc * taps:]
        self._memo_f[key] = out
        return out


AFTER_BACKBONE = None
MIRROR = None


def linear_fwd(x2d, weight, bias=None, relu=False, resid=None, out_scale=1.0, out=None):
    M, K = x2d.shape
    N = weight.shape[0]
    y = out if out is not None else torch.empty((M, N), device=x2d.device, dtype=torch.float32)
    sp = MIRROR.lookup_fwd(weight) if MIRROR is not None else None
    gemm_raw(x2d, x2d.stride(0), weight, weight.stride(0), y, y.stride(0), M, N, K, bias=bias, relu=relu,
             resid=resid, ldr=(resid.stride(0) if resid is not None else 0), out_scale=out_scale, B_split=sp)
    return y


def linear_dgrad(dy2d, weight, gate=None, resid=None, dy16=None, twin=False):
    M, N = dy2d.shape
    K = weight.shape[1]
    dx = torch.empty((M, K), device=dy2d.device, dtype=torch.float32)
    m = MIRROR.lookup(weight) if MIRROR is not None else None
    if m is not None:
        dx16 = torch.empty((M, K), device=dy2d.device, dtype=torch.bfloat16) if twin else None
        gemm_raw(dy2d, dy2d.stride(0), m[0], m[1], dx, K, M, K, N, b_layout=0,
                 gate=gate, ldg=(gate.stride(0) if gate is not None else 0),
                 resid=resid, ldr=(resid.stride(0) if resid is not None else 0), B_split=m[2], B16=m[3], precision=bwd_precision(),
                 A16=dy16, C16=dx16)
        return (dx, dx16) if twin else dx
    gemm_raw(dy2d, dy2d.stride(0), weight, weight.stride(0), dx, K, M, K, N, b_layout=1,
             gate=gate, ldg=(gate.stride(0) if gate is not None else 0),
             resid=resid, ldr=(resid.stride(0) if resid is not None else 0), precision=bwd_precision())
    return (dx, None) if twin else dx


class LinearFn(torch.autograd.Function):

    @staticmethod
    def forward(ctx, x, wparam, bparam, lo, hi, relu, resid, out_scale):
        shp = x.shape
        w = wparam.detach()[lo:hi]
        b = bparam.detach()[lo:hi] if bparam is not None else None
        x2d = x.reshape(-1, shp[-1])
        if x2d.stride(-1) != 1 or (x2d.stride(0) & 3) or (x2d.data_ptr() & 15):
            x2d = x2d.contiguous()
        r2d = None
        if resid is not None:
            r2d = resid.reshape(-1, w.shape[0])
            if r2d.stride(-1) != 1:
                r2d = r2d.contiguous()
        y = linear_fwd(x2d, w, b, relu, r2d, out_scale)
        ctx.relu, ctx.out_scale, ctx.has_resid, ctx.lo, ctx.hi = relu, out_scale, resid is not None, lo, hi
        ctx.wparam, ctx.bparam = wparam, bparam
        ctx.save_for_backward(x2d, y if relu else None)
        ctx.xshape = shp
        return y.reshape(*shp[:-1], w.shape[0])

    @staticmethod
    def backward(ctx, dy):
        x2d, y = ctx.saved_tensors
        wparam, bparam, lo, hi = ctx.wparam, ctx.bparam, ctx.lo, ctx.hi
        w = wparam.detach()[lo:hi]
        dy2d = dy.reshape(-1, w.shape[0])
        if not dy2d.is_contiguous():
            dy2d = dy2d.contiguous()
        if ctx.relu:
            if ctx.has_resid:
                dy2d = relu_mask(y, dy2d)
                d_resid = dy2d.reshape(dy.shape)
                if ctx.out_scale != 1.0:
                    dy2d = dy2d * ctx.out_scale
            else:
                dy2d = relu_mask(y, dy2d, ctx.out_scale)
                d_resid = None
        else:
            d_resid = dy2d.reshape(dy.shape) if ctx.has_resid else None
            if ctx.out_scale != 1.0:
                dy2d = dy2d * ctx.out_scale
        dx = None
        if ctx.needs_input_grad[0]:
            dx = linear_dgrad(dy2d, w).reshape(ctx.xshape)
        if wparam.requires_grad:
            gw = grad_buffer(wparam)[lo:hi]
            gb = grad_buffer(bparam)[lo:hi] if (bparam is not None and bparam.requires_grad) else None
            wgrad_raw(dy2d, dy2d.stride(0), x2d, x2d.stride(0), gw, gw.stride(0), dy2d.shape[0], w.shape[0], x2d.shape[1],
                      dbias=gb, may_defer=True)
        return dx, None, None, None, None, None, d_resid, None


class PosMlpFn(torch.autograd.Function):

    @staticmethod
    def forward(ctx, w0, b0, w2, b2, *xs):
        W0, B0, W2, B2 = w0.detach(), b0.detach(), w2.detach(), b2.detach()
        x2 = []
        for x in xs:
            t = x.reshape(-1, x.shape[-1])
            if t.stride(-1) != 1 or (t.stride(0) & 3) or (t.data_ptr() & 15):
                t = t.contiguous()
            x2.append(t)
        with gemm_queue():
            hs = [linear_fwd(t, W0, B0, relu=True) for t in x2]
        with gemm_queue():
            ys = [linear_fwd(h, W2, B2) for h in hs]
        ctx.params = (w0, b0, w2, b2)
        ctx.n = len(xs)
        ctx.shapes = [x.shape for x in xs]
        ctx.save_for_backward(*x2, *hs)
        return tuple(y.reshape(*x.shape[:-1], y.shape[-1]) for y, x in zip(ys, xs))

    @staticmethod
    def backward(ctx, *dys):
        n = ctx.n
        saved = ctx.saved_tensors
        x2, hs = saved[:n], saved[n:]
        w0, b0, w2, b2 = ctx.params
# ... 292 lines not shown
               and bwd_precision() == 3 and Cout % 64 == 0 and Cin % 64 == 0 and Nb * Hin * Win > 1024)
    assert dz is not None or (m is not None and dz16 is not None), "a gradient that exists as a twin only needs the weight images"
    dx = out if out is not None else (None if no_fp32 else torch.empty((Nb, Hin, Win, Cin), device=dz16.device if dz is None else dz.device, dtype=torch.float32))
    dx16 = torch.empty((Nb, Hin, Win, Cin), device=(dz16 if dz is None else dz).device, dtype=torch.bfloat16) if twin else None
    if m is not None:
        gemm_raw(dz, Cout, m[0], m[1], dx, Cin, Nb * Hin * Win, Cin, Cout, taps=kh * kw, b_layout=0,
                 gate=gate, ldg=Cin, resid=resid, ldr=Cin, geom=g, B_split=m[2], B16=m[3], precision=bwd_precision(), C16=dx16, A16=dz16,
                 gate16=gate16 if gate is not None else None, prio=DGRAD_PRIO, gate16_only=g16_only)
    else:
        gemm_raw(dz, Cout, weight, Cin, dx, Cin, Nb * Hin * Win, Cin, Cout, taps=kh * kw, b_layout=1, w_scale=scale,
                 gate=gate, ldg=Cin, resid=resid, ldr=Cin, geom=g, precision=bwd_precision(), C16=dx16)
    return (dx, dx16) if twin else dx


def conv_wgrad_(dz, x, weight, scale, stride=1, pad=0, dil=1, dz16=None, x16=None):
    Nb, Ho, Wo, Cout = (dz if dz is not None else dz16).shape
    _, H, W, Cin = x.shape
    kh, kw = weight.shape[2:]
    g, Ho2, Wo2 = conv_geom_fwd(H, W, kh, kw, stride, pad, dil)
    assert (Ho2, Wo2) == (Ho, Wo)
    if isinstance(x, Groups):
        assert x16 is not None and dz16 is not None and bwd_precision() == 3 and Cout % 8 == 0 and Cin % 8 == 0 and Nb * Ho * Wo > 1024, \
            "a grouped activation feeds a weight gradient through its bf16 twin"
        x = None
    gw = grad_buffer(weight)
    assert gw.is_contiguous(memory_format=torch.channels_last) or (kh == 1 and kw == 1)
    wgrad_raw(dz, Cout, x, Cin, gw, kh * kw * Cin, Nb * Ho * Wo, Cout, Cin, taps=kh * kw, w_scale=scale, geom=g, may_defer=True,
              dY16=dz16, X16=x16)


def maxpool3x3s2(x, split=False):
    Nb, H, W, Cc = x.shape
    Ho, Wo = (H - 1) // 2 + 1, (W - 1) // 2 + 1
    y = torch.empty((Nb, Ho, Wo, Cc), device=x.device, dtype=torch.float32)
    if split:
        yh = torch.empty((Nb, Ho, Wo, Cc), device=x.device, dtype=torch.bfloat16)
        yl = torch.empty((Nb, Ho, Wo, Cc), device=x.device, dtype=torch.bfloat16)
        check(lib().cdetr_maxpool3x3s2_split(ptr(x), ptr(y), ptr(yh), ptr(yl), Nb, H, W, Cc, stream_ptr()), "cdetr_maxpool3x3s2_split")
        return y, yh, yl
    check(lib().cdetr_maxpool3x3s2(ptr(x), ptr(y), Nb, H, W, Cc, stream_ptr()), "cdetr_maxpool3x3s2")
    return y


RCDA_SKIP_SAVE = os.environ.get("CDETR_RCDA_SKIP_SAVE", "1") != "0"
RCDA_SAVE = True
RCDA_SLICES = os.environ.get("CDETR_RCDA_SLICES", "1") != "0"
FUSE_RCDA_DQ = os.environ.get("CDETR_RCDA_FUSE_DQ", "1") != "0"
FUSE_RCDA_DK = os.environ.get("CDETR_RCDA_FUSE_DK", "1") != "0"


def rcda_pads(H, W):
    return (H + 7) & ~7, (W + 3) & ~3


def rcda_fwd_raw(q_row, q_col, k_row, k_col, v, mask_row, mask_col, nh, save=None):
    N, L, E = q_row.shape
    H, W = v.shape[1:3]
    assert E == nh * 32, "the RCDA kernels are specialised for head_dim 32"
    Hp, Wp = rcda_pads(H, W)
    if save is None:
        save = RCDA_SAVE or not RCDA_SKIP_SAVE
    out = torch.empty((N, L, E), device=v.device, dtype=torch.float32)
    a_row = torch.empty((N, nh, L, Wp), device=v.device, dtype=torch.float32) if save else None
    a_col = torch.empty((N, nh, L, Hp), device=v.device, dtype=torch.float32) if save else None
    d = RcdaFwdDesc()
    d.N, d.L, d.H, d.W, d.nh, d.scale = N, L, H, W, nh, 32 ** -0.5
    d.precision = PRECISION
    d.q_row, d.q_col, d.k_row, d.k_col, d.v = ptr(q_row), ptr(q_col), ptr(k_row), ptr(k_col), ptr(v)
    d.mask_row, d.mask_col = ptr(mask_row), ptr(mask_col)
    d.out, d.a_row, d.a_col = ptr(out), ptr(a_row), ptr(a_col)
    if RCDA_SLICES:
        d.ws, d.ws_bytes = ptr(splitk_ws()), SPLITK_BYTES
    fl = 2.0 * N * nh * L * (H * W * 32 + (H + W) * 32)
    with _Timed("rcda_fwd", fl, None,
                4.0 * N * (3 * L * E + (H + W) * E + H * W * E + nh * L * (Hp + Wp)), fl * _TERMS[d.precision]):
        check(lib().cdetr_rcda_fwd(C.byref(d), stream_ptr()), "cdetr_rcda_fwd")
    return out, a_row, a_col


def rcda_zero_numel(v, k_row, k_col):
    return v.numel() + k_row.numel() + k_col.numel()


def rcda_bwd_raw(d_out, q_row, q_col, k_row, k_col, v, a_row, a_col, nh, zbuf=None):
    N, L, E = q_row.shape
    H, W = v.shape[1:3]
    Hp, Wp = rcda_pads(H, W)
    d_out = d_out.contiguous()
    if zbuf is None:
        zbuf = torch.zeros(rcda_zero_numel(v, k_row, k_col), device=v.device, dtype=torch.float32)
    d_v = zbuf[:v.numel()].view(v.shape)
    d = RcdaBwdDesc()
    d.N, d.L, d.H, d.W, d.nh, d.scale = N, L, H, W, nh, 32 ** -0.5
    d.precision = (3 if bwd_precision() == 3 else 1) if PRECISION == 1 else PRECISION
    d.d_out, d.a_row, d.a_col, d.v = ptr(d_out), ptr(a_row), ptr(a_col), ptr(v)
    d.d_v = ptr(d_v)
    dq_row = torch.empty_like(q_row)
    dq_col = torch.empty_like(q_col)
    fuse_dq = FUSE_RCDA_DQ
    fuse_dk = fuse_dq and FUSE_RCDA_DK and PRECISION == 1
    dk = zbuf[v.numel():]
    dk_row, dk_col = dk[:k_row.numel()].view(k_row.shape), dk[k_row.numel():].view(k_col.shape)
    if fuse_dq:
        d.k_row, d.k_col, d.dq_row, d.dq_col = ptr(k_row), ptr(k_col), ptr(dq_row), ptr(dq_col)
    if fuse_dk:
        d.q_row, d.q_col, d.dk_row, d.dk_col = ptr(q_row), ptr(q_col), ptr(dk_row), ptr(dk_col)
        ds_row = ds_col = None
    else:
        ds_row, ds_col = torch.empty_like(a_row), torch.empty_like(a_col)
        d.ds_row, d.ds_col = ptr(ds_row), ptr(ds_col)
    fl = 2.0 * N * nh * L * (2 * H * W * 32)
    with _Timed("rcda_bwd", fl, None,
                4.0 * N * (5 * L * E + 2 * (H + W) * E + 2 * H * W * E + nh * L * (Hp + Wp)), fl * _TERMS[d.precision]):
        check(lib().cdetr_rcda_bwd(C.byref(d), stream_ptr()), "cdetr_rcda_bwd")
    if not fuse_dq:
        gemm_raw(ds_row, Wp, k_row, E, dq_row, E, L, 32, W, b_layout=1, batch=N * nh, sA=L * Wp, sB=32, sC=32,
                 batch_inner=nh, sA2=nh * L * Wp, sB2=W * E, sC2=L * E)
        gemm_raw(ds_col, Hp, k_col, E, dq_col, E, L, 32, H, b_layout=1, batch=N * nh, sA=L * Hp, sB=32, sC=32,
                 batch_inner=nh, sA2=nh * L * Hp, sB2=H * E, sC2=L * E)
    if not fuse_dk:
        wgrad_raw(ds_row, Wp, q_row, E, dk_row, E, L, W, 32, batch=N * nh, sY=L * Wp, sX=32, sW=32,
                  batch_inner=nh, sY2=nh * L * Wp, sX2=L * E, sW2=W * E)
        wgrad_raw(ds_col, Hp, q_col, E, dk_col, E, L, H, 32, batch=N * nh, sY=L * Hp, sX=32, sW=32,
                  batch_inner=nh, sY2=nh * L * Hp, sX2=L * E, sW2=H * E)
    return dq_row, dq_col, dk_row, dk_col, d_v


class RcdaCoreFn(torch.autograd.Function):

    @staticmethod
    def forward(ctx, q_row, q_col, k_row, k_col, v, mask_row, mask_col, nh):
        q_row, q_col, k_row, k_col, v = [t.contiguous() for t in (q_row, q_col, k_row, k_col, v)]
        out, a_row, a_col = rcda_fwd_raw(q_row, q_col, k_row, k_col, v, mask_row, mask_col, nh)
        ctx.save_for_backward(q_row, q_col, k_row, k_col, v, a_row, a_col)
        ctx.nh = nh
        return out

    @staticmethod
    def backward(ctx, d_out):
        q_row, q_col, k_row, k_col, v, a_row, a_col = ctx.saved_tensors
        return rcda_bwd_raw(d_out, q_row, q_col, k_row, k_col, v, a_row, a_col, ctx.nh) + (None, None, None)


def rcda_core(q_row, q_col, k_row, k_col, v, mask_row, mask_col, nh):
    return RcdaCoreFn.apply(q_row, q_col, k_row, k_col, v, mask_row, mask_col, nh)


def _check_lens(lens, N, device):
    if lens.dtype != torch.int32 or tuple(lens.shape) != (N,) or lens.device != device or not lens.is_contiguous():
        raise ValueError(f"lens must be a contiguous int32 tensor [{N}] on {device}, got {lens.dtype} {tuple(lens.shape)} on {lens.device}")
    return lens


def mha_fwd_raw(qk, v, nh, lens=None):
    N, L, E2 = qk.shape
    E = E2 // 2
    o = torch.empty((N, L, E), device=qk.device, dtype=torch.float32)
    lse = torch.empty((N, nh, L), device=qk.device, dtype=torch.float32)
    if lens is not None:
        check(lib().cdetr_mha_fwd_lens(ptr(qk), ptr(v), ptr(_check_lens(lens, N, qk.device)), ptr(o), ptr(lse), N, L, nh, (E // nh) ** -0.5,
                                       PRECISION, stream_ptr()), "cdetr_mha_fwd_lens")
        return o, lse
    check(lib().cdetr_mha_fwd(ptr(qk), ptr(v), ptr(o), ptr(lse), N, L, nh, (E // nh) ** -0.5, PRECISION, stream_ptr()), "cdetr_mha_fwd")
    return o, lse


def mha_bwd_raw(qk, v, o, d_o, lse, nh, lens=None):
    N, L, E2 = qk.shape
    E = E2 // 2
    d_qk = torch.empty_like(qk)
    d_v = torch.empty_like(v)
    work = torch.empty((N, nh, L), device=qk.device, dtype=torch.float32)
    prec = bwd_precision() if MHA_BWD_BF16 else PRECISION
    if lens is not None:
        check(lib().cdetr_mha_bwd_lens(ptr(qk), ptr(v), ptr(_check_lens(lens, N, qk.device)), ptr(o), ptr(d_o), ptr(lse), ptr(d_qk), ptr(d_v),
                                       ptr(work), N, L, nh, (E // nh) ** -0.5, prec, stream_ptr()), "cdetr_mha_bwd_lens")
        return d_qk, d_v
    check(lib().cdetr_mha_bwd(ptr(qk), ptr(v), ptr(o), ptr(d_o), ptr(lse), ptr(d_qk), ptr(d_v), ptr(work), N, L, nh,
                              (E // nh) ** -0.5, prec, stream_ptr()), "cdetr_mha_bwd")
    return d_qk, d_v


class MhaCoreFn(torch.autograd.Function):

    @staticmethod
    def forward(ctx, qk, v, nh, lens=None):
        assert qk.shape[-1] == 2 * nh * 32, "the MHA kernels are specialised for head_dim 32"
        qk, v = qk.contiguous(), v.contiguous()
        o, lse = mha_fwd_raw(qk, v, nh, lens)
        ctx.save_for_backward(qk, v, o, lse)
        ctx.nh, ctx.lens = nh, lens
        return o

    @staticmethod
    def backward(ctx, d_o):
        qk, v, o, lse = ctx.saved_tensors
        d_qk, d_v = mha_bwd_raw(qk, v, o, d_o.contiguous(), lse, ctx.nh, ctx.lens)
        return d_qk, d_v, None, None


def mha_core(qk, v, nh, lens=None):
    return MhaCoreFn.apply(qk, v, nh, lens)


def _attn_rows(t):
    N, L, E = t.shape
    ld = t.stride(1) if L > 1 else (t.stride(0) if N > 1 else E)
# ... 171 lines not shown


def posadd2(X, Prow, Pcol):
    N, H, W, Cc = X.shape
    Qr, Qc = torch.empty_like(X), torch.empty_like(X)
    check(lib().cdetr_posadd2(ptr(X), ptr(Prow), ptr(Pcol), ptr(Qr), ptr(Qc), N, H, W, Cc, stream_ptr()), "cdetr_posadd2")
    return Qr, Qc


def posadd2_hw_reduce(X, Prow, Pcol):
    N, H, W, Cc = X.shape
    Qr, Qc = torch.empty_like(X), torch.empty_like(X)
    Kr = torch.empty((N, W, Cc), device=X.device, dtype=torch.float32)
    Kc = torch.empty((N, H, Cc), device=X.device, dtype=torch.float32)
    check(lib().cdetr_posadd2_hw_reduce(ptr(X), ptr(Prow), ptr(Pcol), ptr(Qr), ptr(Qc), ptr(Kr), ptr(Kc), N, H, W, Cc, 1.0 / H, 1.0 / W,
                                        stream_ptr()), "cdetr_posadd2_hw_reduce")
    return Qr, Qc, Kr, Kc


def hw_reduce(Xr, Xc, Ar, Ac, scale_r, scale_c):
    N, H, W, Cc = Xr.shape
    Or = torch.empty((N, W, Cc), device=Xr.device, dtype=torch.float32)
    Oc = torch.empty((N, H, Cc), device=Xr.device, dtype=torch.float32)
    check(lib().cdetr_hw_reduce(ptr(Xr), ptr(Xc), ptr(Ar), ptr(Ac), ptr(Or), ptr(Oc), N, H, W, Cc, scale_r, scale_c, stream_ptr()),
          "cdetr_hw_reduce")
    return Or, Oc


def bcast_add2_sum(T, T2, T3, Br, Bc, sr, sc):
    N, H, W, Cc = T.shape
    out = torch.empty_like(T)
    check(lib().cdetr_bcast_add2_sum(ptr(T), ptr(T2), ptr(T3), ptr(Br), ptr(Bc), ptr(out), N, H, W, Cc, sr, sc, stream_ptr()), "cdetr_bcast_add2_sum")
    return out


def bcast_add2(T, Br, Bc, sr, sc):
    N, H, W, Cc = T.shape
    out = torch.empty_like(T)
    check(lib().cdetr_bcast_add2(ptr(T), ptr(Br), ptr(Bc), ptr(out), N, H, W, Cc, sr, sc, stream_ptr()), "cdetr_bcast_add2")
    return out


def _wg(dy2d, x2d, wparam, bparam, lo, hi):
    if not wparam.requires_grad:
        return
    gw = grad_buffer(wparam)[lo:hi]
    gb = grad_buffer(bparam)[lo:hi] if (bparam is not None and bparam.requires_grad) else None
    wgrad_raw(dy2d, dy2d.stride(0), x2d, x2d.stride(0), gw, gw.stride(0), dy2d.shape[0], hi - lo, x2d.shape[1], dbias=gb,
              may_defer=True)


class EncoderLayerFn(torch.autograd.Function):

    @staticmethod
    def forward(ctx, src, posemb_row, posemb_col, mask_row, mask_col, layer, anchor):
        N, H, W, Cc = src.shape
        R = N * H * W
        att = layer.self_attn
        E, nh = att.embed_dim, att.num_heads
        Wi, bi = att.in_proj_weight.detach(), att.in_proj_bias.detach()
        X = src.contiguous()
        Prow, Pcol = posemb_row.contiguous(), posemb_col.contiguous()
        Qr, Qc, Kr, Kc = posadd2_hw_reduce(X, Prow, Pcol)
        with gemm_queue():
            q_row = linear_fwd(Qr.view(R, Cc), Wi[0:E], bi[0:E]).view(N, H * W, E)
            q_col = linear_fwd(Qc.view(R, Cc), Wi[E:2 * E], bi[E:2 * E]).view(N, H * W, E)
            k_row = linear_fwd(Kr.view(N * W, Cc), Wi[2 * E:3 * E], bi[2 * E:3 * E]).view(N, W, E)
            k_col = linear_fwd(Kc.view(N * H, Cc), Wi[3 * E:4 * E], bi[3 * E:4 * E]).view(N, H, E)
            v = linear_fwd(X.view(R, Cc), Wi[4 * E:5 * E], bi[4 * E:5 * E]).view(N, H, W, E)
        o, a_row, a_col = rcda_fwd_raw(q_row, q_col, k_row, k_col, v, mask_row, mask_col, nh)
        Y1 = linear_fwd(o.view(R, E), att.out_proj.weight.detach(), att.out_proj.bias.detach(), resid=X.view(R, Cc))
        X1, mu1, rs1 = ln_fwd_raw(Y1, layer.norm1.weight.detach(), layer.norm1.bias.detach(), layer.norm1.eps)
        f = layer.ffn
        Hd = linear_fwd(X1, f.linear1.weight.detach(), f.linear1.bias.detach(), relu=True)
        Y2 = linear_fwd(Hd, f.linear2.weight.detach(), f.linear2.bias.detach(), resid=X1)
        X2, mu2, rs2 = ln_fwd_raw(Y2, f.norm2.weight.detach(), f.norm2.bias.detach(), f.norm2.eps)
        ctx.save_for_backward(X, Qr, Qc, Kr, Kc, q_row, q_col, k_row, k_col, v, a_row, a_col, o, Y1, mu1, rs1, X1, Hd, Y2, mu2, rs2)
        ctx.layer, ctx.dims = layer, (N, H, W, Cc, E, nh)
        return X2.view(N, H, W, Cc)

    @staticmethod
    def backward(ctx, dX2):
        with wgrad_queue():
            return EncoderLayerFn._backward(ctx, dX2)

    @staticmethod
    def _backward(ctx, dX2, accR=None, accC=None, zbuf=None, defer_out=False):
        (X, Qr, Qc, Kr, Kc, q_row, q_col, k_row, k_col, v, a_row, a_col, o, Y1, mu1, rs1, X1, Hd, Y2, mu2, rs2) = ctx.saved_tensors
        layer = ctx.layer
        N, H, W, Cc, E, nh = ctx.dims
        R = N * H * W
        att, f = layer.self_attn, layer.ffn
        Wi = att.in_proj_weight.detach()
        Wip, bip = att.in_proj_weight, att.in_proj_bias
        ln2 = (Y2, mu2, rs2, f.norm2.weight.detach(), grad_buffer(f.norm2.weight), grad_buffer(f.norm2.bias))
        tw = ENC_TWINS and bf16_twins() and MIRROR is not None
        if isinstance(dX2, tuple):
            pt, pt2, pt3, pKr, pKc = dX2
            dY2 = ln_bwd_raw(pt, *ln2, merge=(pt2, pt3, None, None), bcast=(pKr, pKc, 1.0 / H, 1.0 / W, H, W), twin=tw)
        else:
            dY2 = ln_bwd_raw(dX2.reshape(R, Cc).contiguous(), *ln2, twin=tw)
        dY2, dY2h = dY2 if tw else (dY2, None)
        _wg(dY2, Hd, f.linear2.weight, f.linear2.bias, 0, Cc)
        dHd = linear_dgrad(dY2, f.linear2.weight.detach(), gate=Hd, dy16=dY2h, twin=tw)
        dHd, dHdh = dHd if tw else (dHd, None)
        _wg(dHd, X1, f.linear1.weight, f.linear1.bias, 0, Hd.shape[1])
        dX1 = linear_dgrad(dHd, f.linear1.weight.detach(), resid=dY2, dy16=dHdh)
        dY1 = ln_bwd_raw(dX1, Y1, mu1, rs1, layer.norm1.weight.detach(), grad_buffer(layer.norm1.weight), grad_buffer(layer.norm1.bias), twin=tw)
        dY1, dY1h = dY1 if tw else (dY1, None)
        o2d = o.view(R, E)
        _wg(dY1, o2d, att.out_proj.weight, att.out_proj.bias, 0, Cc)
        dO = linear_dgrad(dY1, att.out_proj.weight.detach(), dy16=dY1h).view(N, H * W, E)
        dq_row, dq_col, dk_row, dk_col, dv = rcda_bwd_raw(dO, q_row, q_col, k_row, k_col, v, a_row, a_col, nh, zbuf)
        dq_row2, dq_col2, dv2 = dq_row.view(R, E), dq_col.view(R, E), dv.view(R, E)
        dk_row2, dk_col2 = dk_row.view(N * W, E), dk_col.view(N * H, E)
        _wg(dq_row2, Qr.view(R, Cc), Wip, bip, 0, E)
        _wg(dq_col2, Qc.view(R, Cc), Wip, bip, E, 2 * E)
        _wg(dk_row2, Kr.view(N * W, Cc), Wip, bip, 2 * E, 3 * E)
        _wg(dk_col2, Kc.view(N * H, Cc), Wip, bip, 3 * E, 4 * E)
        _wg(dv2, X.view(R, Cc), Wip, bip, 4 * E, 5 * E)
        with gemm_queue():
            t = linear_dgrad(dq_row2, Wi[0:E], resid=dY1)
            t2 = linear_dgrad(dq_col2, Wi[E:2 * E])
            t3 = linear_dgrad(dv2, Wi[4 * E:5 * E])
            dKr = linear_dgrad(dk_row2, Wi[2 * E:3 * E])
            dKc = linear_dgrad(dk_col2, Wi[3 * E:4 * E])
            dKrA = linear_dgrad(dk_row2, Wi[2 * E:3 * E], resid=accR.reshape(N * W, Cc)) if accR is not None else dKr
            dKcA = linear_dgrad(dk_col2, Wi[3 * E:4 * E], resid=accC.reshape(N * H, Cc)) if accC is not None else dKc
        dX = (t, t2, t3, dKr, dKc) if defer_out else bcast_add2_sum(t.view(N, H, W, Cc), t2.view(N, H, W, Cc), t3.view(N, H, W, Cc), dKr, dKc,
                                                                    1.0 / H, 1.0 / W)
        sr, sc = hw_reduce(dq_row.view(N, H, W, E), dq_col.view(N, H, W, E), None, None, 1.0, 1.0)
        with gemm_queue():
            dProw = linear_dgrad(sr.view(N * W, E), Wi[0:E], resid=dKrA).view(N, W, Cc)
            dPcol = linear_dgrad(sc.view(N * H, E), Wi[E:2 * E], resid=dKcA).view(N, H, Cc)
        return dX, dProw, dPcol, None, None, None, None


class EncoderStackFn(torch.autograd.Function):

    @staticmethod
    def forward(ctx, src, posemb_row, posemb_col, mask_row, mask_col, layers, anchor, taps):
        x = src
        ctxs = []
        for li, layer in enumerate(layers):
            c = _Ctx()
            x = EncoderLayerFn.forward(c, x, posemb_row, posemb_col, mask_row, mask_col, layer, None)
            ctxs.append(c)
            if taps is not None:
                taps[f"enc{li}"] = x.detach()
        ctx.ctxs = ctxs
        ctx.set_materialize_grads(False)
        return x, posemb_row.view_as(posemb_row), posemb_col.view_as(posemb_col)

    @staticmethod
    def backward(ctx, dX, dPR=None, dPC=None):
        accR = dPR.contiguous() if dPR is not None else None
        accC = dPC.contiguous() if dPC is not None else None
        c0 = ctx.ctxs[0]
        N, H, W, Cc, E, nh = c0.dims
        zn = N * H * W * E + N * W * E + N * H * E
        zall = zeros_flat(len(ctx.ctxs) * zn, dX.device)
        with wgrad_queue():
            for li in range(len(ctx.ctxs) - 1, -1, -1):
                c = ctx.ctxs[li]
                dX, accR, accC = EncoderLayerFn._backward(c, dX, accR, accC, zall[li * zn:(li + 1) * zn], defer_out=(li > 0 and ENC_DEFER))[:3]
                c.saved_tensors = None
        ctx.ctxs = None
        return dX, accR, accC, None, None, None, None, None


class _Ctx:

    def save_for_backward(self, *ts):
        self.saved_tensors = ts

    def set_materialize_grads(self, flag):
        pass


def add2(T, A, B=None):
    O1 = torch.empty_like(T)
    O2 = torch.empty_like(T) if B is not None else None
    check(lib().cdetr_add2(ptr(T), ptr(A), ptr(B), ptr(O1), ptr(O2), T.numel(), stream_ptr()), "cdetr_add2")
    return O1, O2


def grad_merge(base, g1, g2=None, acc1=None, acc2=None):
    out = torch.empty_like(base)
    check(lib().cdetr_grad_merge(ptr(base), ptr(g1), ptr(g2), ptr(acc1), ptr(acc2), ptr(out), base.numel(), stream_ptr()),
          "cdetr_grad_merge")
    return out


class DecoderStackFn(torch.autograd.Function):

    @staticmethod
    def forward(ctx, tgt, qpos, qx, qy, memory, krm, kcm, mask_row, mask_col, layers, anchor, posemb_row=None, posemb_col=None, lens=None):
        N, L, E = tgt.shape
        ctx.lens = lens
        _, H, W, _ = memory.shape
        M = N * L
        tgt, qpos, qx, qy = tgt.contiguous(), qpos.contiguous(), qx.contiguous(), qy.contiguous()
        memory = memory.contiguous()
        mem2 = memory.view(N * H * W, E)
        ctx.own_means = krm is None
        if ctx.own_means:
            krm, kcm = hw_reduce(memory, memory, posemb_row.contiguous(), posemb_col.contiguous(), 1.0 / H, 1.0 / W)
        krm2, kcm2 = krm.contiguous().view(N * W, E), kcm.contiguous().view(N * H, E)
        outs = []
        saved = []
        x = tgt.view(M, E)
        mem_side = []
        with gemm_queue():
            for layer in layers:
                ca = layer.cross_attn
                Wc, bc = ca.in_proj_weight.detach(), ca.in_proj_bias.detach()
                mem_side.append((linear_fwd(krm2, Wc[2 * E:3 * E], bc[2 * E:3 * E]).view(N, W, E),
                                 linear_fwd(kcm2, Wc[3 * E:4 * E], bc[3 * E:4 * E]).view(N, H, E),
                                 linear_fwd(mem2, Wc[4 * E:5 * E], bc[4 * E:5 * E]).view(N, H, W, E)))
        a1_next = None
        for li, layer in enumerate(layers):
            sa, ca, f = layer.self_attn, layer.cross_attn, layer.ffn
            nh = sa.num_heads
            Ws, bs = sa.in_proj_weight.detach(), sa.in_proj_bias.detach()
            Wc, bc = ca.in_proj_weight.detach(), ca.in_proj_bias.detach()
            if a1_next is None:
                a1, _ = add2(x, qpos.view(M, E))
            else:
                a1 = a1_next
            with gemm_queue():
                qk = linear_fwd(a1, Ws[0:2 * E], bs[0:2 * E])
                vs = linear_fwd(x, Ws[2 * E:3 * E], bs[2 * E:3 * E])
            o1, lse = mha_fwd_raw(qk.view(N, L, 2 * E), vs.view(N, L, E), nh, lens)
            Y2 = linear_fwd(o1.view(M, E), sa.out_proj.weight.detach(), sa.out_proj.bias.detach(), resid=x)
            T1, mu2, rs2, qr_in, qc_in = ln_fwd_add_raw(Y2, layer.norm2.weight.detach(), layer.norm2.bias.detach(), layer.norm2.eps,
                                                        qx.view(M, E), qy.view(M, E))
            with gemm_queue():
                q_row = linear_fwd(qr_in, Wc[0:E], bc[0:E]).view(N, L, E)
                q_col = linear_fwd(qc_in, Wc[E:2 * E], bc[E:2 * E]).view(N, L, E)
            k_row, k_col, v = mem_side[li]
            o2, a_row, a_col = rcda_fwd_raw(q_row, q_col, k_row, k_col, v, mask_row, mask_col, ca.num_heads)
            Y1 = linear_fwd(o2.view(M, E), ca.out_proj.weight.detach(), ca.out_proj.bias.detach(), resid=T1)
            T2, mu1, rs1 = ln_fwd_raw(Y1, layer.norm1.weight.detach(), layer.norm1.bias.detach(), layer.norm1.eps)
            Hd = linear_fwd(T2, f.linear1.weight.detach(), f.linear1.bias.detach(), relu=True)
            Y3 = linear_fwd(Hd, f.linear2.weight.detach(), f.linear2.bias.detach(), resid=T2)
            if li + 1 < len(layers):
                out, mu3, rs3, a1_next, _ = ln_fwd_add_raw(Y3, f.norm2.weight.detach(), f.norm2.bias.detach(), f.norm2.eps, qpos.view(M, E))
            else:
                out, mu3, rs3 = ln_fwd_raw(Y3, f.norm2.weight.detach(), f.norm2.bias.detach(), f.norm2.eps)
            outs.append(out.view(N, L, E))
            saved.append((x, a1, qk, vs, o1, lse, Y2, mu2, rs2, T1, qr_in, qc_in, q_row, q_col, k_row, k_col, v, a_row, a_col, o2,
                          Y1, mu1, rs1, T2, Hd, Y3, mu3, rs3))
            x = out
        ctx.layers, ctx.saved, ctx.dims = layers, saved, (N, L, E, H, W)
        ctx.shared = (mem2, krm2, kcm2)
        ctx.set_materialize_grads(False)
        return tuple(outs)

    @staticmethod
    def backward(ctx, *d_outs):
        with wgrad_queue():
            return DecoderStackFn._backward(ctx, *d_outs)

    @staticmethod
    def _backward(ctx, *d_outs):
        layers, saved = ctx.layers, ctx.saved
        N, L, E, H, W = ctx.dims
        mem2, krm2, kcm2 = ctx.shared
        M = N * L
        dev = mem2.device
        zn = N * H * W * E + N * W * E + N * H * E
        zall = zeros_flat(3 * M * E + len(layers) * zn, dev)
        acc = zall[:3 * M * E].view(3, M, E)
        acc_p, acc_x, acc_y = acc[0], acc[1], acc[2]
        dMem = dKrm = dKcm = None
        pend_t = pend_g = None
        for li in range(len(layers) - 1, -1, -1):
            layer = layers[li]
            sa, ca, f = layer.self_attn, layer.cross_attn, layer.ffn
            (x, a1, qk, vs, o1, lse, Y2, mu2, rs2, T1, qr_in, qc_in, q_row, q_col, k_row, k_col, v, a_row, a_col, o2,
             Y1, mu1, rs1, T2, Hd, Y3, mu3, rs3) = saved[li]
            saved[li] = None
            g_out = d_outs[li].reshape(M, E).contiguous() if d_outs[li] is not None else None
            Ws, Wc = sa.in_proj_weight.detach(), ca.in_proj_weight.detach()
            ln3 = (Y3, mu3, rs3, f.norm2.weight.detach(), grad_buffer(f.norm2.weight), grad_buffer(f.norm2.bias))
            if pend_t is None:
                if g_out is None:
                    continue
                dY3 = ln_bwd_raw(g_out, *ln3)
            else:
                dY3 = ln_bwd_raw(pend_t, *ln3, merge=(pend_g, g_out, acc_p, None))
            _wg(dY3, Hd, f.linear2.weight, f.linear2.bias, 0, E)
            dHd = linear_dgrad(dY3, f.linear2.weight.detach(), gate=Hd)
            _wg(dHd, T2, f.linear1.weight, f.linear1.bias, 0, Hd.shape[1])
            dT2 = linear_dgrad(dHd, f.linear1.weight.detach(), resid=dY3)
            dY1 = ln_bwd_raw(dT2, Y1, mu1, rs1, layer.norm1.weight.detach(), grad_buffer(layer.norm1.weight), grad_buffer(layer.norm1.bias))
            _wg(dY1, o2.view(M, E), ca.out_proj.weight, ca.out_proj.bias, 0, E)
            dO2 = linear_dgrad(dY1, ca.out_proj.weight.detach()).view(N, L, E)
            dq_row, dq_col, dk_row, dk_col, dv = rcda_bwd_raw(dO2, q_row, q_col, k_row, k_col, v, a_row, a_col, ca.num_heads,
                                                              zall[3 * M * E + li * zn:3 * M * E + (li + 1) * zn])
            dq_row2, dq_col2 = dq_row.view(M, E), dq_col.view(M, E)
            dk_row2, dk_col2, dv2 = dk_row.view(N * W, E), dk_col.view(N * H, E), dv.view(N * H * W, E)
            Wcp, bcp = ca.in_proj_weight, ca.in_proj_bias
            _wg(dq_row2, qr_in, Wcp, bcp, 0, E)
            _wg(dq_col2, qc_in, Wcp, bcp, E, 2 * E)
            _wg(dk_row2, krm2, Wcp, bcp, 2 * E, 3 * E)
            _wg(dk_col2, kcm2, Wcp, bcp, 3 * E, 4 * E)
            _wg(dv2, mem2, Wcp, bcp, 4 * E, 5 * E)
            with gemm_queue():
                gx = linear_dgrad(dq_row2, Wc[0:E])
                gy = linear_dgrad(dq_col2, Wc[E:2 * E])
                dKrm = linear_dgrad(dk_row2, Wc[2 * E:3 * E], resid=dKrm)
                dKcm = linear_dgrad(dk_col2, Wc[3 * E:4 * E], resid=dKcm)
                dMem = linear_dgrad(dv2, Wc[4 * E:5 * E], resid=dMem)
            dY2 = ln_bwd_raw(dY1, Y2, mu2, rs2, layer.norm2.weight.detach(), grad_buffer(layer.norm2.weight), grad_buffer(layer.norm2.bias),
                             merge=(gx, gy, acc_x, acc_y))
            _wg(dY2, o1.view(M, E), sa.out_proj.weight, sa.out_proj.bias, 0, E)
            dO1 = linear_dgrad(dY2, sa.out_proj.weight.detach()).view(N, L, E)
            dqk, dvs = mha_bwd_raw(qk.view(N, L, 2 * E), vs.view(N, L, E), o1, dO1, lse, sa.num_heads, ctx.lens)
            Wsp, bsp = sa.in_proj_weight, sa.in_proj_bias
            _wg(dqk.view(M, 2 * E), a1, Wsp, bsp, 0, 2 * E)
            _wg(dvs.view(M, E), x, Wsp, bsp, 2 * E, 3 * E)
            with gemm_queue():
                ga1 = linear_dgrad(dqk.view(M, 2 * E), Ws[0:2 * E])
                t = linear_dgrad(dvs.view(M, E), Ws[2 * E:3 * E], resid=dY2)
            pend_t, pend_g = t, ga1
        dx = grad_merge(pend_t, pend_g, None, acc_p, None)
        if ctx.own_means:
            dMem = bcast_add2(dMem.view(N, H, W, E), dKrm, dKcm, 1.0 / H, 1.0 / W)
            return (dx.view(N, L, E), acc_p.view(N, L, E), acc_x.view(N, L, E), acc_y.view(N, L, E), dMem, None, None, None, None, None,
                    None, dKrm.view(N, W, E), dKcm.view(N, H, E), None)
        return (dx.view(N, L, E), acc_p.view(N, L, E), acc_x.view(N, L, E), acc_y.view(N, L, E), dMem.view(N, H, W, E),
                dKrm.view(N, W, E), dKcm.view(N, H, E), None, None, None, None, None, None, None)


class MatchPlan:

    def __init__(self, sizes, Q, device, _capacity=None):
        self.Q = Q
        self.device = device
        self.Tcap = _capacity
        if _capacity is None:
            self._set_host(sizes)
            coff = [0]
            for s in self.sizes:
                coff.append(coff[-1] + Q * s)
            self.tgt_off = torch.tensor(self.tgt_off_host, dtype=torch.int32, device=device)
            self.sizes_f = torch.tensor([float(s) for s in self.sizes], dtype=torch.float32, device=device)
            self.Mmax = max(max(self.M), 1)
            self.nc_max = max([Q] + self.sizes)
        else:
            B = int(sizes)
            self.B = B
            coff = [b * Q * _capacity for b in range(B + 1)]
            self.tgt_off = torch.zeros(B + 1, dtype=torch.int32, device=device)
            self.sizes_f = torch.zeros(B, dtype=torch.float32, device=device)
            self.Mmax = max(min(Q, _capacity), 1)
            self.nc_max = max(Q, _capacity)
            self._set_host([0] * B)
        self.cost_off = torch.tensor(coff[:-1], dtype=torch.int64, device=device)
        self.cost_numel = max(coff[-1], 1)
        self.cost_off_host = coff

    @classmethod
    def capacity(cls, B, Q, Tcap, device):
        return cls(B, Q, device, _capacity=int(Tcap))

    def _set_host(self, sizes):
        self.sizes = [int(s) for s in sizes]
        self.B = len(self.sizes)
        off = [0]
        for s in self.sizes:
            off.append(off[-1] + s)
        self.tgt_off_host = off
        self.M = [min(self.Q, s) for s in self.sizes]

    def set_counts(self, sizes):
        assert self.Tcap is not None and len(sizes) == self.B and max(sizes, default=0) <= self.Tcap
        self._set_host(sizes)
        self.tgt_off.copy_(torch.tensor(self.tgt_off_host, dtype=torch.int32))
        self.sizes_f.copy_(torch.tensor([float(s) for s in self.sizes], dtype=torch.float32))


class PackedTargets:

    def __init__(self, boxes, labels, plan):
        self.boxes, self.labels, self.plan = boxes, labels, plan

    @classmethod
    def with_capacity(cls, B, Q, Tcap, device):
        return cls(torch.zeros((B * Tcap, 4), dtype=torch.float32, device=device), torch.zeros(B * Tcap, dtype=torch.int64, device=device),
                   MatchPlan.capacity(B, Q, Tcap, device))

    def load(self, targets):
        sizes = [int(t["boxes"].shape[0]) for t in targets]
        n = sum(sizes)
        if n:
            self.boxes[:n].copy_(torch.cat([t["boxes"].reshape(-1, 4) for t in targets]))
            self.labels[:n].copy_(torch.cat([t["labels"].reshape(-1) for t in targets]))
        self.plan.set_counts(sizes)
        return n


def match_cost(logits, boxes, tgt_boxes, plan, w_class=2.0, w_bbox=5.0, w_giou=2.0):
    cost = torch.empty(plan.cost_numel, device=logits.device, dtype=torch.float32)
    logits = logits.contiguous()
    boxes = boxes.contiguous()
    tgt_boxes = tgt_boxes.contiguous()
    check(lib().cdetr_match_cost(ptr(logits), logits.shape[-1], ptr(boxes), ptr(tgt_boxes) if tgt_boxes.numel() else ptr(cost),
                                 ptr(plan.tgt_off), ptr(plan.cost_off), plan.B, plan.Q, w_class, w_bbox, w_giou, ptr(cost),
# ... 447 lines not shown
```

include/cdetr_hip.h:

```cpp
#ifndef CDETR_HIP_H
#define CDETR_HIP_H
#include <stddef.h>
#include <stdint.h>

#ifdef __cplusplus
extern "C" {
#endif

#define CDETR_ABI_VERSION 2

#define CDETR_ROWS_DENSE 0
#define CDETR_ROWS_CONV_FWD 1
#define CDETR_ROWS_CONV_DGRAD 2

typedef struct {
    int32_t mode;
    int32_t Ha, Wa;
    int32_t Hc, Wc;
    int32_t kh, kw, stride, pad, dil;
} cdetr_conv_geom;

typedef struct {
    int32_t M, N, K, taps;
    int32_t batch;
// ... 28 lines not shown
#define CDETR_GEMM_RESID_GROUPS 8
#define CDETR_GEMM_GATE16_ONLY 16
int cdetr_gemm(const cdetr_gemm_desc* d, void* stream);
int cdetr_gemm_dl(const cdetr_gemm_desc* d, int32_t tile, int32_t stages, void* stream);
int cdetr_gemm_group(const cdetr_gemm_desc* descs, int32_t n, void* stream);

typedef struct {
    int32_t P, Nout, Cin, taps;
    int32_t batch;
    int32_t precision;
    const float* dY; int64_t ldy, sY;
    const float* X; int64_t ldx, sX;
    float* dW; int64_t ldw, sW;
    const float* w_scale;
    float* dbias;
    cdetr_conv_geom g;
    int32_t batch_inner;
    int32_t wg_target;
    int64_t sY2, sX2, sW2;
    const void* dY16;
    const void* X16;
} cdetr_wgrad_desc;
int cdetr_wgrad(const cdetr_wgrad_desc* d, void* stream);
int cdetr_wgrad_group(const cdetr_wgrad_desc* descs, int32_t n, void* stream);

int cdetr_colsum(const float* X, int64_t ldx, int32_t M, int32_t N, float* out, void* stream);

#define CDETR_SUMSQ_MAX_BLOCKS 2048
#define CDETR_SUMSQ_WS_FLOATS CDETR_SUMSQ_MAX_BLOCKS
int cdetr_sumsq(const float* g, int64_t n, float* out, float* workspace, void* stream);
int cdetr_adamw_step(float* p, const float* g, float* m, float* v, const float* lr, int64_t n, const float* sumsq,
                     float* state, float max_norm, float beta1, float beta2, float eps, float weight_decay, float grad_div,
                     void* stream);
int cdetr_adamw_step2(float* p, const float* g, float* m, float* v, const float* lr, float lr0, float lr1, int64_t lr_split, int64_t n,
                      const float* sumsq, float* state, float max_norm, float beta1, float beta2, float eps, float weight_decay,
                      float grad_div, void* stream);
int cdetr_sgd_step(float* p, const float* g, float* buf, const float* lr, float lr0, float lr1, int64_t lr_split, int64_t n,
                   const float* sumsq, float* state, float max_norm, float momentum, float weight_decay, float grad_div, void* stream);
int cdetr_relu_mask(const float* y, const float* dy, float* dz, int64_t n, float scale, void* stream);
int cdetr_relu_mask2(const float* y, const float* dy, float* dz, void* dz16, int64_t n, float scale, void* stream);

int cdetr_groupnorm_fwd(const float* x, const float* gamma, const float* beta, float* y, float* mean, float* rstd,
                        int32_t B, int32_t P, int32_t C, int32_t G, float eps, void* stream);
int cdetr_groupnorm_bwd(const float* dy, const float* x, const float* mean, const float* rstd, const float* gamma, float* dx,
                        float* dgamma, float* dbeta, int32_t B, int32_t P, int32_t C, int32_t G, void* stream);
int cdetr_groupnorm_fwd_ws(const float* x, const float* gamma, const float* beta, float* y, float* mean, float* rstd,
                           int32_t B, int32_t P, int32_t C, int32_t G, float eps, void* ws, int64_t ws_bytes, void* stream);
int cdetr_groupnorm_bwd_ws(const float* dy, const float* x, const float* mean, const float* rstd, const float* gamma, float* dx,
                           float* dgamma, float* dbeta, int32_t B, int32_t P, int32_t C, int32_t G, void* ws, int64_t ws_bytes, void* stream);

int cdetr_layernorm_fwd(const float* x, const float* gamma, const float* beta, float* y, float* mean, float* rstd,
                        int32_t rows, int32_t C, float eps, void* stream);
int cdetr_layernorm_fwd_add(const float* x, const float* gamma, const float* beta, float* y, float* mean, float* rstd,
                            const float* a1, const float* a2, float* o1, float* o2, int32_t rows, int32_t C, float eps, void* stream);
int cdetr_layernorm_bwd(const float* dy, const float* x, const float* mean, const float* rstd, const float* gamma,
                        const float* add, float* dx, float* dgamma, float* dbeta, int32_t rows, int32_t C, void* dx16, void* stream);
int cdetr_layernorm_bwd_merge(const float* dy, const float* g1, const float* g2, float* acc1, float* acc2, const float* Br, const float* Bc,
                              float sr, float sc, int32_t H, int32_t W, const float* x, const float* mean, const float* rstd,
                              const float* gamma, const float* add, float* dx, float* dgamma, float* dbeta, int32_t rows, int32_t C,
                              void* dx16, void* stream);
int cdetr_posadd2(const float* X, const float* Prow, const float* Pcol, float* Qr, float* Qc, int32_t N, int32_t H, int32_t W,
                  int32_t C, void* stream);
int cdetr_hw_reduce(const float* Xr, const float* Xc, const float* Ar, const float* Ac, float* Or, float* Oc, int32_t N,
                    int32_t H, int32_t W, int32_t C, float scale_r, float scale_c, void* stream);
int cdetr_posadd2_hw_reduce(const float* X, const float* Prow, const float* Pcol, float* Qr, float* Qc, float* Kr, float* Kc, int32_t N,
                            int32_t H, int32_t W, int32_t C, float scale_r, float scale_c, void* stream);
int cdetr_bcast_add2(const float* T, const float* Br, const float* Bc, float* out, int32_t N, int32_t H, int32_t W, int32_t C,
                     float sr, float sc, void* stream);
int cdetr_bcast_add2_sum(const float* T, const float* T2, const float* T3, const float* Br, const float* Bc, float* out, int32_t N, int32_t H,
                         int32_t W, int32_t C, float sr, float sc, void* stream);
int cdetr_add2(const float* T, const float* A, const float* B, float* O1, float* O2, int64_t n, void* stream);
int cdetr_sine_embed(const float* pos, int32_t pstride, float* out, int64_t ldo, int32_t rows, int32_t nfeat, float temperature,
                     void* stream);
int cdetr_sine_embed_bwd(const float* pos, int32_t pstride, const float* dout, int64_t ldo, float* dpos, int32_t dstride, int32_t rows,
                         int32_t nfeat, float temperature, int32_t accumulate, void* stream);
int cdetr_grad_merge(const float* base, const float* g1, const float* g2, float* acc1, float* acc2, float* out, int64_t n,
                     void* stream);

typedef struct {
    const float* src;
    float* dst;
    void* dst_split;
    const float* scale;
    int32_t R, C, taps, tile0, transpose, pad_;
    void* dst_hi;
} cdetr_mirror_item;
int cdetr_weight_mirror(const cdetr_mirror_item* items_dev, int32_t n_items, int32_t total_tiles, void* stream);
int cdetr_weight_images(const cdetr_mirror_item* items_dev, int32_t n_items, int32_t total_blocks, void* stream);

int cdetr_maxpool3x3s2(const float* X, float* Y, int32_t Nimg, int32_t H, int32_t W, int32_t C, void* stream);
int cdetr_maxpool3x3s2_split(const float* X, float* Y, void* Y16, void* Y16lo, int32_t Nimg, int32_t H, int32_t W, int32_t C, void* stream);

typedef struct {
    int32_t N, L, H, W, nh;
    int32_t precision;
    float scale;
    const float* q_row; const float* q_col; const float* k_row; const float* k_col; const float* v;
    const uint8_t* mask_row; const uint8_t* mask_col;
    float* out; float* a_row; float* a_col;
    void* ws;
    int64_t ws_bytes;
} cdetr_rcda_fwd_desc;
int cdetr_rcda_fwd(const cdetr_rcda_fwd_desc* d, void* stream);

typedef struct {
    int32_t N, L, H, W, nh;
    int32_t precision;
    float scale;
    const float* d_out; const float* a_row; const float* a_col; const float* v;
    float* ds_row; float* ds_col; float* d_v;
    const float* k_row; const float* k_col;
    float* dq_row; float* dq_col;
    const float* q_row; const float* q_col;
    float* dk_row; float* dk_col;
} cdetr_rcda_bwd_desc;
int cdetr_rcda_bwd(const cdetr_rcda_bwd_desc* d, void* stream);
static inline int32_t cdetr_rcda_wp(int32_t W) { return (W + 3) & ~3; }
static inline int32_t cdetr_rcda_hp(int32_t H) { return (H + 7) & ~7; }

int cdetr_mha_fwd(const float* qk, const float* v, float* o, float* lse, int32_t N, int32_t L, int32_t nh, float scale,
                  int32_t precision, void* stream);
int cdetr_mha_bwd(const float* qk, const float* v, const float* o, const float* d_o, const float* lse, float* d_qk, float* d_v,
                  float* work, int32_t N, int32_t L, int32_t nh, float scale, int32_t precision, void* stream);

int cdetr_mha_fwd_lens(const float* qk, const float* v, const int32_t* lens, float* o, float* lse, int32_t N, int32_t L, int32_t nh,
                       float scale, int32_t precision, void* stream);
int cdetr_mha_bwd_lens(const float* qk, const float* v, const int32_t* lens, const float* o, const float* d_o, const float* lse, float* d_qk,
                       float* d_v, float* work, int32_t N, int32_t L, int32_t nh, float scale, int32_t precision, void* stream);

typedef struct {
    const float* q; const float* k; const float* v;
    int64_t ldq, ldk, ldv;
    float* o; float* lse;
    const float* d_o;
    float* d_q; float* d_k; float* d_v;
    int64_t ld_dq, ld_dk, ld_dv;
    float* work;
    int32_t N, Lq, Lk, nh;
    float scale;
    int32_t precision;
} cdetr_attn_desc;
int cdetr_attn_fwd(const cdetr_attn_desc* d, void* stream);
int cdetr_attn_bwd(const cdetr_attn_desc* d, void* stream);

int cdetr_match_cost(const float* logits, int32_t ncls, const float* boxes, const float* tgt, const int32_t* tgt_off,
                     const int64_t* cost_off, int32_t B, int32_t Q, float w_class, float w_bbox, float w_giou,
                     float* cost, void* stream);
int cdetr_lsap(const float* cost, const int64_t* cost_off, const int32_t* tgt_off, int32_t B, int32_t Q,
               int32_t nc_max, int32_t Mmax, int64_t* idx_i, int64_t* idx_j, int32_t* status, void* stream);

typedef struct {
    int32_t B, Q, C, num_classes, Mmax;
    float alpha;
    const float* logits;
    const float* boxes;
    const float* vars;
    const float* tgt_boxes;
    const int64_t* tgt_labels;
    const int32_t* tgt_off;
    const int64_t* idx_i;
    const int64_t* idx_j;
    const float* num_boxes;
    float* losses;
    float* g_logits;
    float* g_l1;
    float* g_giou;
    float* g_var_box;
    float* g_vars;
    const float* loss_weights;
} cdetr_criterion_desc;
int cdetr_criterion_fwd(const cdetr_criterion_desc* d, void* stream);
int cdetr_criterion_bwd(const float* g6, const float* g_total, const float* loss_weights, const float* g_logits, const float* g_l1,
                        const float* g_giou, const float* g_var_box, const float* g_vars, float* d_logits, float* d_boxes, float* d_vars,
                        int32_t BQ, int32_t C, void* stream);

typedef struct {
    int32_t B, Q, C, num_classes, Mmax;
    float alpha;
    const float* logits;
    const float* boxes;
    const float* vars;
    const float* tgt_boxes;
    const int64_t* tgt_labels;
    const int32_t* tgt_off;
    const int64_t* idx_i;
    const int64_t* idx_j;
    float* losses;
    const float* loss_weights;
} cdetr_criterion_eval_desc;
int cdetr_criterion_eval(const cdetr_criterion_eval_desc* d, void* stream);

int cdetr_bbox_criterion_fwd(const float* pred_wh, int64_t pred_stride, const float* tgt_points, const float* tgt_whs, int32_t M,
                             float w_wh, float w_giou, float* losses, float* g_wh, float* g_giou, void* stream);
int cdetr_bbox_criterion_bwd(const float* g3, float w_wh, float w_giou, const float* g_wh, const float* g_giou, float* d_coord,
                             int32_t M, void* stream);

int cdetr_bbox_criterion_lens_fwd(const float* pred_wh, int64_t pred_stride, const float* tgt_points, const float* tgt_whs,
// ... 116 lines not shown
```

Baseline: 246.8 images/s.

## Stack decoder cross-attn K/V dgrads into one wide GEMM and group direct GEMMs

```diff
diff --git a/counting_detr_amd/_ffi.py b/counting_detr_amd/_ffi.py
--- a/counting_detr_amd/_ffi.py
+++ b/counting_detr_amd/_ffi.py
@@ -46,7 +46,8 @@
     _fields_ = [("N", C.c_int32), ("L", C.c_int32), ("H", C.c_int32), ("W", C.c_int32), ("nh", C.c_int32),
                 ("precision", C.c_int32), ("scale", C.c_float), ("d_out", _p), ("a_row", _p), ("a_col", _p), ("v", _p),
                 ("ds_row", _p), ("ds_col", _p), ("d_v", _p), ("k_row", _p), ("k_col", _p), ("dq_row", _p), ("dq_col", _p),
-                ("q_row", _p), ("q_col", _p), ("dk_row", _p), ("dk_col", _p)]
+                ("q_row", _p), ("q_col", _p), ("dk_row", _p), ("dk_col", _p),
+                ("ld_dv", C.c_int64), ("ld_dk_row", C.c_int64), ("ld_dk_col", C.c_int64)]
 
 
 class AttnDesc(C.Structure):
@@ -71,7 +72,7 @@
 
 class MirrorItem(C.Structure):
     _fields_ = [("src", _p), ("dst", _p), ("dst_split", _p), ("scale", _p), ("R", C.c_int32), ("C", C.c_int32), ("taps", C.c_int32),
-                ("tile0", C.c_int32), ("transpose", C.c_int32), ("pad_", C.c_int32), ("dst_hi", _p)]
+                ("tile0", C.c_int32), ("transpose", C.c_int32), ("dst_ld", C.c_int32), ("dst_hi", _p)]
 
 
 class CocoMatchDesc(C.Structure):
diff --git a/counting_detr_amd/csrc/elementwise.hip b/counting_detr_amd/csrc/elementwise.hip
--- a/counting_detr_amd/csrc/elementwise.hip
+++ b/counting_detr_amd/csrc/elementwise.hip
@@ -178,6 +178,7 @@
     const int r0 = (t / tilesC) * 32, c0 = (t % tilesC) * 32;
     const int tx = threadIdx.x & 31, ty = threadIdx.x >> 5;
     __bf16* sp = reinterpret_cast<__bf16*>(it.dst_split);
+    const long ldk = it.dst_ld ? it.dst_ld : it.taps * it.R;
     float vin[4], sin_[4];
     const int cc = min(c0 + tx, it.C - 1);
 #pragma unroll
@@ -208,11 +209,11 @@
         const int c = c0 + ty + 8 * p, r = r0 + tx;
         if (r < it.R && c < it.C) {
             const float v = tile[tx][ty + 8 * p];
-            if (it.dst) it.dst[((long)c * it.taps + tap) * it.R + r] = v;
-            if (it.dst_hi) reinterpret_cast<__bf16*>(it.dst_hi)[((long)c * it.taps + tap) * it.R + r] = (__bf16)v;
+            if (it.dst) it.dst[(long)c * ldk + tap * it.R + r] = v;
+            if (it.dst_hi) reinterpret_cast<__bf16*>(it.dst_hi)[(long)c * ldk + tap * it.R + r] = (__bf16)v;
             if (sp) {
                 const __bf16 h = (__bf16)v;
-                __bf16* g = sp + (long)c * it.taps * it.R * 2 + (long)((tap * it.R + r0) >> 5) * 64;
+                __bf16* g = sp + (long)c * ldk * 2 + (long)((tap * it.R + r0) >> 5) * 64;
                 g[tx] = h;
                 g[32 + tx] = (__bf16)(v - (float)h);
             }
diff --git a/counting_detr_amd/csrc/igemm.hip b/counting_detr_amd/csrc/igemm.hip
--- a/counting_detr_amd/csrc/igemm.hip
+++ b/counting_detr_amd/csrc/igemm.hip
@@ -1624,6 +1624,16 @@
     igemm_direct_body<BL, UB>(it.d, it.tilesM, it.tilesN, it.vecA, it.vecB, lb % it.nx, lb / it.nx);
 }
 
+__global__ __launch_bounds__(256) void igemm_direct_multi_group_kernel(const GemmGroupArgs g) {
+    int p = 0;
+    while (p + 1 < g.n && (int)blockIdx.x >= g.blk0[p + 1]) ++p;
+    const GemmGroupItem& it = g.it[p];
+    const int lb = blockIdx.x - g.blk0[p];
+    if (it.pad_ == 0) igemm_direct_body<0, 4>(it.d, it.tilesM, it.tilesN, it.vecA, it.vecB, lb % it.nx, lb / it.nx);
+    else if (it.pad_ == 1) igemm_direct_body<0, 8>(it.d, it.tilesM, it.tilesN, it.vecA, it.vecB, lb % it.nx, lb / it.nx);
+    else igemm_direct_body<0, 16>(it.d, it.tilesM, it.tilesN, it.vecA, it.vecB, lb % it.nx, lb / it.nx);
+}
+
 template <int TERMS>
 __global__ __launch_bounds__(512) void igemm_mixed_group_kernel(const GemmGroupArgs g) {
     int p = 0;
@@ -2074,6 +2084,26 @@
         if (int rcl = cdetr_launch_status("cdetr_gemm_group")) return rcl;
         cls[0].clear();
         cls[tc].clear();
+    }
+    if (((int)!cls[0].empty() + (int)!cls[1].empty() + (int)!cls[2].empty()) >= 2 && cls[0].size() + cls[1].size() + cls[2].size() <= (size_t)GG_MAX) {
+        GemmGroupArgs g;
+        int m = 0;
+        g.blk0[0] = 0;
+        for (int c = 2; c >= 0; --c) {
+            for (int idx : cls[c]) {
+                GemmGroupItem& it = g.it[m];
+                it.d = descs[idx];
+                it.vecA = gemm_vec_a(it.d); it.vecB = gemm_vec_b(it.d); it.pad_ = c;
+                it.tilesM = (it.d.M + 15) / 16; it.tilesN = (it.d.N + 15) / 16;
+                it.nx = it.tilesM * it.tilesN;
+                g.blk0[m + 1] = g.blk0[m] + it.nx * it.d.batch;
+                ++m;
+            }
+            cls[c].clear();
+        }
+        g.n = m;
+        hipLaunchKernelGGL(igemm_direct_multi_group_kernel, dim3(g.blk0[m]), dim3(256), 0, st, g);
+        if (int rcl = cdetr_launch_status("cdetr_gemm_group")) return rcl;
     }
     for (int c = 0; c < 5; ++c) {
         for (size_t c0 = 0; c0 < cls[c].size(); c0 += GG_MAX) {
diff --git a/counting_detr_amd/csrc/rcda.hip b/counting_detr_amd/csrc/rcda.hip
--- a/counting_detr_amd/csrc/rcda.hip
+++ b/counting_detr_amd/csrc/rcda.hip
@@ -985,7 +985,8 @@
                     const float* S = side == 0 ? dArow : Acol;
                     float* Sw = side == 0 ? dArow : Acol;
                     const int sstr = side == 0 ? sm.sw : sm.sh;
-                    float* acc_g = (side == 0 ? d.dk_row + (long)n * W * E : d.dk_col + (long)n * H * E) + head * D + i32;
+                    const long ldk = side == 0 ? d.ld_dk_row : d.ld_dk_col;
+                    float* acc_g = (side == 0 ? d.dk_row + (long)n * W * ldk : d.dk_col + (long)n * H * ldk) + head * D + i32;
                     bf16x8 bh[2], bl[2];
 #pragma unroll
                     for (int st = 0; st < 2; ++st) {
@@ -1034,7 +1035,7 @@
 #pragma unroll
                             for (int r = 0; r < 16; ++r) {
                                 const int wk = 32 * tl + (r & 3) + 8 * (r >> 2) + 4 * g;
-                                if (wk < nkeys) atomicAdd(acc_g + (long)wk * E, acc[r]);
+                                if (wk < nkeys) atomicAdd(acc_g + (long)wk * ldk, acc[r]);
                             }
                         }
                     }
@@ -1051,7 +1052,7 @@
 #pragma unroll
                         for (int wv = 0; wv < NW; ++wv) sum += base[wv * wstr];
                         const int key = idx >> 5, ch = idx & 31;
-                        float* dst = rowside ? d.dk_row + ((long)n * W + key) * E + head * D + ch : d.dk_col + ((long)n * H + key) * E + head * D + ch;
+                        float* dst = rowside ? d.dk_row + ((long)n * W + key) * d.ld_dk_row + head * D + ch : d.dk_col + ((long)n * H + key) * d.ld_dk_col + head * D + ch;
                         atomicAdd(dst, sum);
                     }
                 }
@@ -1193,7 +1194,7 @@
 #pragma unroll
         for (int r = 0; r < 16; ++r) {
             const int h = 32 * f + (r & 3) + 8 * (r >> 2) + 4 * g;
-            if (h < H) atomicAdd(d.d_v + (((long)n * H + h) * W + w) * E + head * D + i32, acc[f][r]);
+            if (h < H) atomicAdd(d.d_v + (((long)n * H + h) * W + w) * d.ld_dv + head * D + i32, acc[f][r]);
         }
 }
 
@@ -1330,7 +1331,7 @@
 #pragma unroll
         for (int r = 0; r < 16; ++r) {
             const int wl = 32 * f + (r & 3) + 8 * (r >> 2) + 4 * g, w = wbase + wl;
-            if (wl < Wc && w < W) atomicAdd(d.d_v + (((long)n * H + h) * W + w) * E + head * D + i32, acc[f][r]);
+            if (wl < Wc && w < W) atomicAdd(d.d_v + (((long)n * H + h) * W + w) * d.ld_dv + head * D + i32, acc[f][r]);
         }
 }
 
@@ -1489,7 +1490,7 @@
 
 extern "C" int cdetr_rcda_bwd(const cdetr_rcda_bwd_desc* dp, void* stream) {
     CDETR_CHECK_ARG(dp != nullptr, "cdetr_rcda_bwd: null descriptor");
-    const cdetr_rcda_bwd_desc d = *dp;
+    cdetr_rcda_bwd_desc d = *dp;
     CDETR_CHECK_ARG(d.N > 0 && d.L > 0 && d.H > 0 && d.W > 0 && d.nh > 0, "cdetr_rcda_bwd: bad sizes");
     CDETR_CHECK_ARG(d.H <= 128 && d.W <= 1024, "cdetr_rcda_bwd: H must be <= 128 (got %d)", d.H);
     CDETR_CHECK_ARG(d.d_out && d.a_row && d.a_col && d.v && d.d_v, "cdetr_rcda_bwd: null pointer");
@@ -1498,6 +1499,14 @@
     CDETR_CHECK_ARG(!d.dq_row || (d.dq_col && d.k_row && d.k_col), "cdetr_rcda_bwd: dq_row needs dq_col, k_row and k_col");
     CDETR_CHECK_ARG(!d.dk_row || (d.dq_row && d.dk_col && d.q_row && d.q_col && d.precision >= 1),
                     "cdetr_rcda_bwd: dk_row needs dk_col, q_row, q_col, the dq_* outputs and a split-bf16 precision (1 or 3)");
+    const int64_t E = (int64_t)d.nh * D;
+    if (!d.ld_dv) d.ld_dv = E;
+    if (!d.ld_dk_row) d.ld_dk_row = E;
+    if (!d.ld_dk_col) d.ld_dk_col = E;
+    CDETR_CHECK_ARG(d.ld_dv >= E && d.ld_dk_row >= E && d.ld_dk_col >= E, "cdetr_rcda_bwd: ld_dv / ld_dk_row / ld_dk_col must be 0 or >= E = %d", (int)E);
+    CDETR_CHECK_ARG(d.ld_dv % 4 == 0 && d.ld_dk_row % 4 == 0 && d.ld_dk_col % 4 == 0 && (reinterpret_cast<uintptr_t>(d.d_v) & 15) == 0 &&
+                    (reinterpret_cast<uintptr_t>(d.dk_row) & 15) == 0 && (reinterpret_cast<uintptr_t>(d.dk_col) & 15) == 0,
+                    "cdetr_rcda_bwd: d_v / dk_row / dk_col must be 16-byte aligned with row strides that are multiples of 4 floats");
     hipStream_t st = reinterpret_cast<hipStream_t>(stream);
     const int NF = d.H <= 32 ? 1 : (d.H <= 64 ? 2 : 4);
     const int Wp = (d.W + 3) & ~3;
diff --git a/counting_detr_amd/engine.py b/counting_detr_amd/engine.py
--- a/counting_detr_amd/engine.py
+++ b/counting_detr_amd/engine.py
@@ -183,7 +183,15 @@
                 entries.append((p.data, None))
             if p.shape[1] % 32 == 0:
                 fwd.append((p.data, None))
-    return ops.WeightMirror(entries, fwd) if (entries or fwd) else None
+    stacks = []
+    for m in model.modules() if (dgrad and entries) else ():
+        ws = [l.cross_attn.in_proj_weight.data for l in getattr(m, "decoder_layers", ()) if hasattr(getattr(l, "cross_attn", None), "in_proj_weight")]
+        if not ws or len(ws) != len(m.decoder_layers) or not all(w.is_cuda and w.is_contiguous() for w in ws):
+            continue
+        E = ws[0].shape[1]
+        if all(tuple(w.shape) == (5 * E, E) for w in ws) and E % 32 == 0:
+            stacks += [[w[i * E:(i + 1) * E] for w in ws] for i in (2, 3, 4)]
+    return ops.WeightMirror(entries, fwd, stacks) if (entries or fwd) else None
 
 
 class _DeviceEvents:
diff --git a/counting_detr_amd/ops.py b/counting_detr_amd/ops.py
--- a/counting_detr_amd/ops.py
+++ b/counting_detr_amd/ops.py
@@ -394,7 +394,7 @@
 
 class WeightMirror:
 
-    def __init__(self, entries, fwd_entries=()):
+    def __init__(self, entries, fwd_entries=(), stacks=()):
         import bisect
         import numpy as np
         self._bisect = bisect
@@ -406,10 +406,11 @@
         self.flat_t16 = torch.zeros(max(tot_t, 1), device=dev, dtype=torch.bfloat16)
         self.flat_fs = torch.zeros(max(tot_f, 1), device=dev, dtype=torch.float32)
         self._keep = []
-        items = (MirrorItem * (len(entries) + len(fwd_entries)))()
+        n_stacked = sum(len(st) for st in stacks)
+        items = (MirrorItem * (len(entries) + n_stacked + len(fwd_entries)))()
         self.t_entries, self.f_entries = [], []
         tile0 = 0
-        self.nT = len(entries)
+        self.nT = len(entries) + n_stacked
 
         def geom(w):
             R, Cc = w.shape[0], w.shape[1]
@@ -434,13 +435,35 @@
             self._keep.append((w, sc))
             tile0 += ((R + 31) // 32) * ((Cc + 31) // 32) * taps
             off += w.numel()
+        tot_s = sum(sum(w.numel() for w in st) for st in stacks)
+        self.stk = torch.zeros(max(tot_s, 1), device=dev, dtype=torch.float32)
+        self.stk_s = torch.zeros(max(tot_s, 1), device=dev, dtype=torch.float32)
+        self.stk_16 = torch.zeros(max(tot_s, 1), device=dev, dtype=torch.bfloat16)
+        self._stacks = {}
+        i, off = len(entries), 0
+        for st in stacks:
+            R, Cc = st[0].shape
+            ldk = len(st) * R
+            assert R % 32 == 0 and all(w.dim() == 2 and tuple(w.shape) == (R, Cc) and w.is_contiguous() for w in st)
+            for l, w in enumerate(st):
+                it = items[i]
+                k0 = l * R
+                it.src, it.dst = w.data_ptr(), self.stk.data_ptr() + 4 * (off + k0)
+                it.dst_split, it.dst_hi = self.stk_s.data_ptr() + 4 * (off + k0), self.stk_16.data_ptr() + 2 * (off + k0)
+                it.scale = None
+                it.R, it.C, it.taps, it.tile0, it.transpose, it.dst_ld = R, Cc, 1, tile0, 1, ldk
+                self._keep.append((w, None))
+                tile0 += (R // 32) * ((Cc + 31) // 32)
+                i += 1
+            self._stacks[tuple(w.data_ptr() for w in st)] = (self.stk[off:], ldk, self.stk_s[off:], self.stk_16[off:])
+            off += ldk * Cc
         self.tilesT = tile0
         tile0 = 0
         off = 0
         for j, (w, sc) in enumerate(fwd_entries):
             R, Cc, taps = geom(w)
             assert Cc % 32 == 0
-            it = items[len(entries) + j]
+            it = items[self.nT + j]
             it.src, it.dst, it.dst_split = w.data_ptr(), None, self.flat_fs.data_ptr() + 4 * off
             it.scale = sc.data_ptr() if sc is not None else None
             it.R, it.C, it.taps, it.tile0, it.transpose = R, Cc, taps, tile0, 0
@@ -493,6 +516,9 @@
         self._memo_t[key] = out
         return out
 
+    def lookup_stack(self, ws):
+        return self._stacks.get(tuple(w.data_ptr() for w in ws))
+
     def lookup_fwd(self, w, scale=None):
         key = (w.data_ptr(), scale.data_ptr() if scale is not None else 0)
         hit = self._memo_f.get(key, False)
@@ -538,6 +564,21 @@
              gate=gate, ldg=(gate.stride(0) if gate is not None else 0),
              resid=resid, ldr=(resid.stride(0) if resid is not None else 0), precision=bwd_precision())
     return (dx, None) if twin else dx
+
+
+def stacked_dgrad(dys, weights, ld=None):
+    M = dys.shape[0]
+    Nout, K = weights[0].shape
+    n = len(weights)
+    ld = dys.stride(0) if ld is None else ld
+    dx = torch.empty((M, K), device=dys.device, dtype=torch.float32)
+    m = MIRROR.lookup_stack(weights) if MIRROR is not None else None
+    if m is not None:
+        gemm_raw(dys, ld, m[0], m[1], dx, K, M, K, n * Nout, b_layout=0, B_split=m[2], B16=m[3], precision=bwd_precision())
+    else:
+        Wcat = torch.cat([w.reshape(Nout, K) for w in weights], 0)
+        gemm_raw(dys, ld, Wcat, K, dx, K, M, K, n * Nout, b_layout=1, precision=bwd_precision())
+    return dx
 
 
 class LinearFn(torch.autograd.Function):
@@ -996,15 +1037,25 @@
     return v.numel() + k_row.numel() + k_col.numel()
 
 
-def rcda_bwd_raw(d_out, q_row, q_col, k_row, k_col, v, a_row, a_col, nh, zbuf=None):
+def rcda_bwd_raw(d_out, q_row, q_col, k_row, k_col, v, a_row, a_col, nh, zbuf=None, into=None):
     N, L, E = q_row.shape
     H, W = v.shape[1:3]
     Hp, Wp = rcda_pads(H, W)
     d_out = d_out.contiguous()
-    if zbuf is None:
-        zbuf = torch.zeros(rcda_zero_numel(v, k_row, k_col), device=v.device, dtype=torch.float32)
-    d_v = zbuf[:v.numel()].view(v.shape)
+    if into is not None:
+        d_v, dk_row, dk_col = into
+        assert d_v.shape == v.shape and dk_row.shape == k_row.shape and dk_col.shape == k_col.shape
+        ld_v, ld_r, ld_c = d_v.stride(2), dk_row.stride(1), dk_col.stride(1)
+        assert d_v.stride() == (H * W * ld_v, W * ld_v, ld_v, 1) and dk_row.stride() == (W * ld_r, ld_r, 1) and dk_col.stride() == (H * ld_c, ld_c, 1)
+    else:
+        if zbuf is None:
+            zbuf = torch.zeros(rcda_zero_numel(v, k_row, k_col), device=v.device, dtype=torch.float32)
+        d_v = zbuf[:v.numel()].view(v.shape)
+        dk = zbuf[v.numel():]
+        dk_row, dk_col = dk[:k_row.numel()].view(k_row.shape), dk[k_row.numel():].view(k_col.shape)
+        ld_v = ld_r = ld_c = E
     d = RcdaBwdDesc()
+    d.ld_dv, d.ld_dk_row, d.ld_dk_col = ld_v, ld_r, ld_c
     d.N, d.L, d.H, d.W, d.nh, d.scale = N, L, H, W, nh, 32 ** -0.5
     d.precision = (3 if bwd_precision() == 3 else 1) if PRECISION == 1 else PRECISION
     d.d_out, d.a_row, d.a_col, d.v = ptr(d_out), ptr(a_row), ptr(a_col), ptr(v)
@@ -1013,8 +1064,6 @@
     dq_col = torch.empty_like(q_col)
     fuse_dq = FUSE_RCDA_DQ
     fuse_dk = fuse_dq and FUSE_RCDA_DK and PRECISION == 1
-    dk = zbuf[v.numel():]
-    dk_row, dk_col = dk[:k_row.numel()].view(k_row.shape), dk[k_row.numel():].view(k_col.shape)
     if fuse_dq:
         d.k_row, d.k_col, d.dq_row, d.dq_col = ptr(k_row), ptr(k_col), ptr(dq_row), ptr(dq_col)
     if fuse_dk:
@@ -1033,10 +1082,10 @@
         gemm_raw(ds_col, Hp, k_col, E, dq_col, E, L, 32, H, b_layout=1, batch=N * nh, sA=L * Hp, sB=32, sC=32,
                  batch_inner=nh, sA2=nh * L * Hp, sB2=H * E, sC2=L * E)
     if not fuse_dk:
-        wgrad_raw(ds_row, Wp, q_row, E, dk_row, E, L, W, 32, batch=N * nh, sY=L * Wp, sX=32, sW=32,
-                  batch_inner=nh, sY2=nh * L * Wp, sX2=L * E, sW2=W * E)
-        wgrad_raw(ds_col, Hp, q_col, E, dk_col, E, L, H, 32, batch=N * nh, sY=L * Hp, sX=32, sW=32,
-                  batch_inner=nh, sY2=nh * L * Hp, sX2=L * E, sW2=H * E)
+        wgrad_raw(ds_row, Wp, q_row, E, dk_row, ld_r, L, W, 32, batch=N * nh, sY=L * Wp, sX=32, sW=32,
+                  batch_inner=nh, sY2=nh * L * Wp, sX2=L * E, sW2=W * ld_r)
+        wgrad_raw(ds_col, Hp, q_col, E, dk_col, ld_c, L, H, 32, batch=N * nh, sY=L * Hp, sX=32, sW=32,
+                  batch_inner=nh, sY2=nh * L * Hp, sX2=L * E, sW2=H * ld_c)
     return dq_row, dq_col, dk_row, dk_col, d_v
 
 
@@ -1374,7 +1423,9 @@
     @staticmethod
     def backward(ctx, dX2):
         with wgrad_queue():
-            return EncoderLayerFn._backward(ctx, dX2)
+            dX, (dKr, pR), (dKc, pC) = EncoderLayerFn._backward(ctx, dX2)
+            N, H, W, Cc = ctx.dims[:4]
+            return dX, (dKr + pR).view(N, W, Cc), (dKc + pC).view(N, H, Cc), None, None, None, None
 
     @staticmethod
     def _backward(ctx, dX2, accR=None, accC=None, zbuf=None, defer_out=False):
@@ -1411,21 +1462,22 @@
         _wg(dk_row2, Kr.view(N * W, Cc), Wip, bip, 2 * E, 3 * E)
         _wg(dk_col2, Kc.view(N * H, Cc), Wip, bip, 3 * E, 4 * E)
         _wg(dv2, X.view(R, Cc), Wip, bip, 4 * E, 5 * E)
+        sr, sc = hw_reduce(dq_row.view(N, H, W, E), dq_col.view(N, H, W, E), None, None, 1.0, 1.0)
+        aRk, aRq = accR if accR is not None else (None, None)
+        aCk, aCq = accC if accC is not None else (None, None)
         with gemm_queue():
             t = linear_dgrad(dq_row2, Wi[0:E], resid=dY1)
             t2 = linear_dgrad(dq_col2, Wi[E:2 * E])
             t3 = linear_dgrad(dv2, Wi[4 * E:5 * E])
             dKr = linear_dgrad(dk_row2, Wi[2 * E:3 * E])
             dKc = linear_dgrad(dk_col2, Wi[3 * E:4 * E])
-            dKrA = linear_dgrad(dk_row2, Wi[2 * E:3 * E], resid=accR.reshape(N * W, Cc)) if accR is not None else dKr
-            dKcA = linear_dgrad(dk_col2, Wi[3 * E:4 * E], resid=accC.reshape(N * H, Cc)) if accC is not None else dKc
+            dKrA = linear_dgrad(dk_row2, Wi[2 * E:3 * E], resid=aRk) if aRk is not None else dKr
+            dKcA = linear_dgrad(dk_col2, Wi[3 * E:4 * E], resid=aCk) if aCk is not None else dKc
+            pR = linear_dgrad(sr.view(N * W, E), Wi[0:E], resid=aRq)
+            pC = linear_dgrad(sc.view(N * H, E), Wi[E:2 * E], resid=aCq)
         dX = (t, t2, t3, dKr, dKc) if defer_out else bcast_add2_sum(t.view(N, H, W, Cc), t2.view(N, H, W, Cc), t3.view(N, H, W, Cc), dKr, dKc,
                                                                     1.0 / H, 1.0 / W)
-        sr, sc = hw_reduce(dq_row.view(N, H, W, E), dq_col.view(N, H, W, E), None, None, 1.0, 1.0)
-        with gemm_queue():
-            dProw = linear_dgrad(sr.view(N * W, E), Wi[0:E], resid=dKrA).view(N, W, Cc)
-            dPcol = linear_dgrad(sc.view(N * H, E), Wi[E:2 * E], resid=dKcA).view(N, H, Cc)
-        return dX, dProw, dPcol, None, None, None, None
+        return dX, (dKrA, pR), (dKcA, pC)
 
 
 class EncoderStackFn(torch.autograd.Function):
@@ -1446,19 +1498,19 @@
 
     @staticmethod
     def backward(ctx, dX, dPR=None, dPC=None):
-        accR = dPR.contiguous() if dPR is not None else None
-        accC = dPC.contiguous() if dPC is not None else None
         c0 = ctx.ctxs[0]
         N, H, W, Cc, E, nh = c0.dims
+        accR = (dPR.contiguous().view(N * W, Cc), None) if dPR is not None else None
+        accC = (dPC.contiguous().view(N * H, Cc), None) if dPC is not None else None
         zn = N * H * W * E + N * W * E + N * H * E
         zall = zeros_flat(len(ctx.ctxs) * zn, dX.device)
         with wgrad_queue():
             for li in range(len(ctx.ctxs) - 1, -1, -1):
                 c = ctx.ctxs[li]
-                dX, accR, accC = EncoderLayerFn._backward(c, dX, accR, accC, zall[li * zn:(li + 1) * zn], defer_out=(li > 0 and ENC_DEFER))[:3]
+                dX, accR, accC = EncoderLayerFn._backward(c, dX, accR, accC, zall[li * zn:(li + 1) * zn], defer_out=(li > 0 and ENC_DEFER))
                 c.saved_tensors = None
         ctx.ctxs = None
-        return dX, accR, accC, None, None, None, None, None
+        return dX, (accR[0] + accR[1]).view(N, W, Cc), (accC[0] + accC[1]).view(N, H, Cc), None, None, None, None, None
 
 
 class _Ctx:
@@ -1561,11 +1613,15 @@
         mem2, krm2, kcm2 = ctx.shared
         M = N * L
         dev = mem2.device
+        nl = len(layers)
         zn = N * H * W * E + N * W * E + N * H * E
-        zall = zeros_flat(3 * M * E + len(layers) * zn, dev)
+        zall = zeros_flat(3 * M * E + nl * zn, dev)
         acc = zall[:3 * M * E].view(3, M, E)
         acc_p, acc_x, acc_y = acc[0], acc[1], acc[2]
-        dMem = dKrm = dKcm = None
+        o_r, o_c = 3 * M * E + nl * N * H * W * E, 3 * M * E + nl * (N * H * W * E + N * W * E)
+        dvS = zall[3 * M * E:o_r].view(N, H, W, nl * E)
+        Wcs = [l.cross_attn.in_proj_weight.detach() for l in layers]
+        dkrS, dkcS = zall[o_r:o_c].view(N, W, nl * E), zall[o_c:].view(N, H, nl * E)
         pend_t = pend_g = None
         for li in range(len(layers) - 1, -1, -1):
             layer = layers[li]
@@ -1589,10 +1645,11 @@
             dY1 = ln_bwd_raw(dT2, Y1, mu1, rs1, layer.norm1.weight.detach(), grad_buffer(layer.norm1.weight), grad_buffer(layer.norm1.bias))
             _wg(dY1, o2.view(M, E), ca.out_proj.weight, ca.out_proj.bias, 0, E)
             dO2 = linear_dgrad(dY1, ca.out_proj.weight.detach()).view(N, L, E)
-            dq_row, dq_col, dk_row, dk_col, dv = rcda_bwd_raw(dO2, q_row, q_col, k_row, k_col, v, a_row, a_col, ca.num_heads,
-                                                              zall[3 * M * E + li * zn:3 * M * E + (li + 1) * zn])
+            blk = slice(li * E, (li + 1) * E)
+            dq_row, dq_col = rcda_bwd_raw(dO2, q_row, q_col, k_row, k_col, v, a_row, a_col, ca.num_heads,
+                                          into=(dvS[..., blk], dkrS[..., blk], dkcS[..., blk]))[:2]
             dq_row2, dq_col2 = dq_row.view(M, E), dq_col.view(M, E)
-            dk_row2, dk_col2, dv2 = dk_row.view(N * W, E), dk_col.view(N * H, E), dv.view(N * H * W, E)
+            dk_row2, dk_col2, dv2 = dkrS.view(N * W, nl * E)[:, blk], dkcS.view(N * H, nl * E)[:, blk], dvS.view(N * H * W, nl * E)[:, blk]
             Wcp, bcp = ca.in_proj_weight, ca.in_proj_bias
             _wg(dq_row2, qr_in, Wcp, bcp, 0, E)
             _wg(dq_col2, qc_in, Wcp, bcp, E, 2 * E)
@@ -1602,9 +1659,6 @@
             with gemm_queue():
                 gx = linear_dgrad(dq_row2, Wc[0:E])
                 gy = linear_dgrad(dq_col2, Wc[E:2 * E])
-                dKrm = linear_dgrad(dk_row2, Wc[2 * E:3 * E], resid=dKrm)
-                dKcm = linear_dgrad(dk_col2, Wc[3 * E:4 * E], resid=dKcm)
-                dMem = linear_dgrad(dv2, Wc[4 * E:5 * E], resid=dMem)
             dY2 = ln_bwd_raw(dY1, Y2, mu2, rs2, layer.norm2.weight.detach(), grad_buffer(layer.norm2.weight), grad_buffer(layer.norm2.bias),
                              merge=(gx, gy, acc_x, acc_y))
             _wg(dY2, o1.view(M, E), sa.out_proj.weight, sa.out_proj.bias, 0, E)
@@ -1616,8 +1670,12 @@
             with gemm_queue():
                 ga1 = linear_dgrad(dqk.view(M, 2 * E), Ws[0:2 * E])
                 t = linear_dgrad(dvs.view(M, E), Ws[2 * E:3 * E], resid=dY2)
+                if li == 0:
+                    dKrm = stacked_dgrad(dkrS.view(N * W, nl * E), [w[2 * E:3 * E] for w in Wcs])
+                    dKcm = stacked_dgrad(dkcS.view(N * H, nl * E), [w[3 * E:4 * E] for w in Wcs])
             pend_t, pend_g = t, ga1
         dx = grad_merge(pend_t, pend_g, None, acc_p, None)
+        dMem = stacked_dgrad(dvS.view(N * H * W, nl * E), [w[4 * E:5 * E] for w in Wcs])
         if ctx.own_means:
             dMem = bcast_add2(dMem.view(N, H, W, E), dKrm, dKcm, 1.0 / H, 1.0 / W)
             return (dx.view(N, L, E), acc_p.view(N, L, E), acc_x.view(N, L, E), acc_y.view(N, L, E), dMem, None, None, None, None, None,
diff --git a/include/cdetr_hip.h b/include/cdetr_hip.h
--- a/include/cdetr_hip.h
+++ b/include/cdetr_hip.h
@@ -134,7 +134,8 @@
     float* dst;
     void* dst_split;
     const float* scale;
-    int32_t R, C, taps, tile0, transpose, pad_;
+    int32_t R, C, taps, tile0, transpose;
+    int32_t dst_ld;
     void* dst_hi;
 } cdetr_mirror_item;
 int cdetr_weight_mirror(const cdetr_mirror_item* items_dev, int32_t n_items, int32_t total_tiles, void* stream);
@@ -165,6 +166,7 @@
     float* dq_row; float* dq_col;
     const float* q_row; const float* q_col;
     float* dk_row; float* dk_col;
+    int64_t ld_dv, ld_dk_row, ld_dk_col;
 } cdetr_rcda_bwd_desc;
 int cdetr_rcda_bwd(const cdetr_rcda_bwd_desc* d, void* stream);
 static inline int32_t cdetr_rcda_wp(int32_t W) { return (W + 3) & ~3; }
```

New measurement: 248.7 images/s (median of 6 runs). No clear change (+0.8%).
